# HAHHHD/mllp

Measured on AMD Instinct MI355X. Metric: LP instances/sec (fwd+bwd) on Netlib batch; achieved HBM GB/s on CSR SpMM, higher is better.
Workload: dtype f32; 1 GPU; netlib_full: BASELINE.json configs[2], 97 instances / 1,074,147 nnz per global batch, one block-diagonal batch per GPU, one Adam step per global batch: fwd + BCE + bwd + gradient all-reduce + Adam, fp32; global_batch=97, instances_rank0=97, nnz_rank0=1074147, hip_graph=False, parallelism=dp1

## Files before the change

mllp_amd/csrc/fused_kernels.hip:

```cpp
#include <algorithm>
#include <vector>

#include "device_utils.h"
#include "host_graph.h"
#include "internal.h"
#include "node_bodies.h"

namespace mllp {

typedef float f32x4m __attribute__((ext_vector_type(4)));

#ifdef MLLP_TIMING_BUILD
static int g_fused_abl = [] {
    const char* e = getenv("MLLP_FUSED_ABL");
    return e ? atoi(e) : 0;
}();
#define FUSED_ABL(bit) ((J.abl & (bit)) != 0)
__device__ unsigned long long g_fused_stamps[8192 * 8];
__device__ unsigned long long g_fused_stamps1[8192 * 8];
#define FUSED_STAMP(k)                                                                      \
    {                                                                                       \
        __builtin_amdgcn_sched_barrier(0);                                                  \
        const unsigned long long now_ = __builtin_amdgcn_s_memtime();                       \
        __builtin_amdgcn_sched_barrier(0);                                                  \
        stamp_sum[k] += now_ - stamp_last;                                                  \
        stamp_last = now_;                                                                  \
    }
#else
#define FUSED_ABL(bit) false
#define FUSED_STAMP(k)
#endif

constexpr int FT = 768;
constexpr int FW = FT / 64;
constexpr int RT = 1024;
constexpr int MAXJOBS = 2;

constexpr int NP = FUSED_NP;
static_assert(NP == FUSED_PARTS, "partition count");

struct PartTiers {
    int row0, n_block, n_wave, n_group, n_base;
};
struct ItemsDev {
    const int* __restrict__ sptr;
    const int2* __restrict__ sent;
    const float2* __restrict__ sax;
    int n_dst, nnz;
    const int* __restrict__ order;
    int nw, L;
    PartTiers part[NP];
};

static ItemsDev items_dev(const FusedOrient& o, int which) {
    const bool scalar = which == 1;
    ItemsDev d;
    d.order = which == 0 ? o.lst16 : which == 1 ? o.lst1 : o.lst16x2;
    d.nw = which == 0 ? o.nw16 : which == 1 ? o.nw1 : o.nw16x2;
    d.L = which == 0 ? o.L16 : which == 1 ? o.L1 : o.L16x2;
    d.sptr = o.sptr;
    d.sent = reinterpret_cast<const int2*>(o.sent);
    d.sax = reinterpret_cast<const float2*>(o.sax);
    d.n_dst = o.n_dst;
    d.nnz = o.nnz;
    for (int q = 0; q < NP; ++q) {
        const FusedTiersDev& t = scalar ? o.t1[q] : o.t16[q];
        d.part[q].row0 = o.row0[q];
        d.part[q].n_block = t.n_block; d.part[q].n_wave = t.n_wave; d.part[q].n_group = t.n_group; d.part[q].n_base = t.n_base;
    }
    return d;
}

constexpr int TS = 17;
constexpr int TILE = 16 * TS;
__device__ __forceinline__ void tile_put(float* tile, const float4& v, int lane) {
    float* d = tile + (lane >> 2) * TS + 4 * (lane & 3);
    d[0] = v.x; d[1] = v.y; d[2] = v.z; d[3] = v.w;
}
__device__ __forceinline__ float4 tile_get(const float* tile, int lane) {
    const float* d = tile + (lane >> 2) * TS + 4 * (lane & 3);
    return make_float4(d[0], d[1], d[2], d[3]);
}
__device__ __forceinline__ void tile_rows(const float* tile, int lane, float (&a)[4]) {
#pragma unroll
    for (int s = 0; s < 4; ++s) a[s] = tile[(lane & 15) * TS + 4 * s + (lane >> 4)];
}
__device__ __forceinline__ void tile_cols(const float* tile, int lane, float (&a)[4]) {
#pragma unroll
    for (int s = 0; s < 4; ++s) a[s] = tile[(4 * s + (lane >> 4)) * TS + (lane & 15)];
}
__device__ __forceinline__ void tile_put_result(float* tile, const f32x4m& d, int lane) {
#pragma unroll
    for (int j = 0; j < 4; ++j) tile[(4 * (lane >> 4) + j) * TS + (lane & 15)] = d[j];
}
struct MatB {
    float w[4];
};
__device__ __forceinline__ MatB matB(const float* __restrict__ W, int ld, int lane) {
    MatB b;
#pragma unroll
    for (int s = 0; s < 4; ++s) b.w[s] = W[(lane & 15) * ld + 4 * s + (lane >> 4)];
    return b;
}
__device__ __forceinline__ MatB matB_t(const float* __restrict__ W, int ld, int lane) {
    MatB b;
#pragma unroll
    for (int s = 0; s < 4; ++s) b.w[s] = W[(4 * s + (lane >> 4)) * ld + (lane & 15)];
    return b;
}
__device__ __forceinline__ void matB_store(float* lds, const MatB& b, int lane) {
    *reinterpret_cast<float4*>(lds + 4 * lane) = make_float4(b.w[0], b.w[1], b.w[2], b.w[3]);
}
__device__ __forceinline__ MatB matB_lds(const float* lds, int lane) {
    const float4 v = *reinterpret_cast<const float4*>(lds + 4 * lane);
    MatB b;
    b.w[0] = v.x; b.w[1] = v.y; b.w[2] = v.z; b.w[3] = v.w;
    return b;
}
__device__ __forceinline__ f32x4m mat_apply(const float (&a)[4], const MatB& b, f32x4m acc) {
#pragma unroll
    for (int s = 0; s < 4; ++s) acc = __builtin_amdgcn_mfma_f32_16x16x4f32(a[s], b.w[s], acc, 0, 0, 0);
    return acc;
}
__device__ __forceinline__ f32x4m splat4(float v) { return (f32x4m){v, v, v, v}; }
__device__ __forceinline__ float4 lds4(const float* p) { return *reinterpret_cast<const float4*>(p); }
__device__ __forceinline__ float4 f4zero() { return make_float4(0.f, 0.f, 0.f, 0.f); }
__device__ __forceinline__ float4 f4scale(const float4& a, float s) { return make_float4(a.x * s, a.y * s, a.z * s, a.w * s); }
__device__ __forceinline__ float4 f4add(const float4& a, const float4& b) { return make_float4(a.x + b.x, a.y + b.y, a.z + b.z, a.w + b.w); }
template <int J>
__device__ __forceinline__ int quad_bcast_i(int v) {
    return __builtin_amdgcn_mov_dpp(v, J * 0x55, 0xF, 0xF, true);
}
__device__ __forceinline__ float wave_sum(float v) {
    v = row16_sum(v);
    v += __shfl_xor(v, 16, 64);
    v += __shfl_xor(v, 32, 64);
    return v;
}


struct RowSlot {
    int row;
    int first;
    int stride;
    int end;
    int mode;
    bool writer;
};
struct SlotReq {
    int row, q, stride, mode;
    int sb, se;
    bool writer;
};
template <int G>
struct Geo {
    static constexpr int U = 64 / G;
    static constexpr int QG = 4;
    static constexpr int RG = U / QG;
};
template <int G>
__device__ __forceinline__ int wave_items(const PartTiers& s) {
    return s.n_wave + (s.n_group + Geo<G>::RG - 1) / Geo<G>::RG + (s.n_base + Geo<G>::U - 1) / Geo<G>::U;
}
template <int G>
__device__ __forceinline__ SlotReq item_request(const ItemsDev& S, const PartTiers& s, int item, int lane) {
    constexpr int U = Geo<G>::U, QG = Geo<G>::QG, RG = Geo<G>::RG;
    const int unit = lane / G;
    const int n_gitems = (s.n_group + RG - 1) / RG;
    SlotReq r;
    bool valid;
    if (item < s.n_wave) {
        r.row = s.row0 + s.n_block + item; r.q = unit; r.stride = U; r.mode = 2; valid = true; r.writer = unit == 0;
    } else if (item < s.n_wave + n_gitems) {
        const int rl = (item - s.n_wave) * RG + unit / QG;
        valid = rl < s.n_group;
        r.row = s.row0 + s.n_block + s.n_wave + rl; r.q = unit % QG; r.stride = QG; r.mode = 1; r.writer = valid && r.q == 0;
    } else {
        const int rl = (item - s.n_wave - n_gitems) * U + unit;
        valid = rl < s.n_base;
        r.row = s.row0 + s.n_block + s.n_wave + s.n_group + rl; r.q = 0; r.stride = 1; r.mode = 0; r.writer = valid;
    }
    const int rc = valid ? r.row : 0;
    r.sb = S.sptr[rc];
    r.se = S.sptr[rc + 1];
    if (!valid) r.row = -1;
    return r;
}
__device__ __forceinline__ SlotReq empty_request() {
    SlotReq r;
    r.row = -1; r.q = 0; r.stride = 1; r.mode = 0; r.sb = 0; r.se = 0; r.writer = false;
    return r;
}
__device__ __forceinline__ RowSlot slot_make(const SlotReq& q) {
    RowSlot r;
    r.row = q.row; r.first = q.sb + q.q; r.stride = q.stride; r.end = q.row >= 0 ? q.se : 0; r.mode = q.mode; r.writer = q.writer;
    asm volatile("" : "+v"(r.first), "+v"(r.end));
    return r;
}
template <int G>
__device__ __forceinline__ RowSlot item_slot(const ItemsDev& S, const PartTiers& s, int item, int lane) {
    return slot_make(item_request<G>(S, s, item, lane));
}
template <int G>
__device__ __forceinline__ RowSlot block_slot(const ItemsDev& s, int k, int tid) {
    RowSlot r;
    r.row = k;
    r.mode = 3;
    r.first = s.sptr[k] + tid / G;
    r.stride = FT / G;
    r.end = s.sptr[k + 1];
    r.writer = tid < G;
    return r;
}
__device__ __forceinline__ int slot_count(const RowSlot& r) {
    return r.first < r.end ? (r.end - r.first + r.stride - 1) / r.stride : 0;
}
__device__ __forceinline__ RowSlot empty_slot() {
    RowSlot r;
    r.row = -1; r.first = 0; r.stride = 1; r.end = 0; r.mode = 0; r.writer = false;
    return r;
}
struct WaveList {
    const int* p;
    int L, chunk;
};
__device__ __forceinline__ WaveList wave_list(const ItemsDev& S, int px, int gw) {
    WaveList w;
    w.L = gw < S.nw ? S.L : 0;
    w.p = S.order + ((size_t)px * S.nw + gw) * S.L;
    w.chunk = -1;
    return w;
}
__device__ __forceinline__ void wave_list_chunk(WaveList& w, int c0, int lane) {
    int v = c0 + lane < w.L ? w.p[c0 + lane] : -1;
    asm volatile("s_waitcnt vmcnt(0)" : "+v"(v));
    w.chunk = v;
}
__device__ __forceinline__ int wave_list_get(const WaveList& w, int k) {
    return k < 64 ? __builtin_amdgcn_readlane(w.chunk, __builtin_amdgcn_readfirstlane(k)) : -1;
}
template <int LPE>
__device__ __forceinline__ int2 first_entries(const ItemsDev& s, const RowSlot& r, int part) {
    const int k = LPE == 4 ? part : (part & 1);
    return k < slot_count(r) ? s.sent[r.first + k * r.stride] : make_int2(0, 0);
}
template <int LPE>
__device__ __forceinline__ int2 first_entries_any(const ItemsDev& s, const RowSlot& r, int part) {
    const int k = LPE == 4 ? part : (part & 1);
    return s.sent[max(min(r.first + k * r.stride, s.nnz - 1), 0)];
}
__device__ __forceinline__ float shared_sum4(float v, int mode) {
    return mode == 1 ? quads_sum<16>(v) : quads_sum<64>(v);
}
__device__ __forceinline__ float shared_max4(float v, int mode) {
    return mode == 1 ? quads_max<16>(v) : quads_max<64>(v);
}
__device__ __forceinline__ float shared_sum1(float v, int mode) { return mode == 1 ? quad_sum(v) : wave_sum(v); }
__device__ __forceinline__ float shared_max1(float v, int mode) { return mode == 1 ? quad_max(v) : group_max<64>(v); }

struct FwdJob16 {
    ItemsDev s;
    const float* __restrict__ x_src;
    const float* __restrict__ x_dst;
    const float* __restrict__ D;
    ConvParams p;
    float* __restrict__ h;
    float* __restrict__ Z;
    float* __restrict__ aux;
    int head;
    const float* __restrict__ fcw;
    const float* __restrict__ fcb;
    const float* __restrict__ inv_n;
    const float* __restrict__ labels;
    const int* __restrict__ perm;
    float inv_batch;
    float* __restrict__ logits;
    float* __restrict__ g_out;
    float* __restrict__ head_part;
#ifdef MLLP_TIMING_BUILD
    int abl;
#endif
};
struct FwdLaunch16 {
    FwdJob16 job[MAXJOBS];
    int n_jobs;
};
struct FwdW16 {
    float BPq[256], BWv[256], BWs[256];
    float pq0[16], Pt[16], bv[16], we[16], bs[16], fcw[16];
    float pt0, fcb;
};
struct SoftState {
    float4 Z;
    float m, L, u;
};

struct Gather4 {
    float4 x0, x1, x2, x3;
    float a0, a1, a2, a3;
};
__device__ __forceinline__ void gather4_issue(const ItemsDev& s, const float* __restrict__ X, const RowSlot& r, int n_mine,
                                              int k0, int part, int2& en, Gather4& g) {
    const int colm = en.x;
    const float am = __int_as_float(en.y);
    const int c0 = quad_bcast_i<0>(colm), c1 = quad_bcast_i<1>(colm), c2 = quad_bcast_i<2>(colm), c3 = quad_bcast_i<3>(colm);
    g.a0 = quad_bcast<0>(am); g.a1 = quad_bcast<1>(am); g.a2 = quad_bcast<2>(am); g.a3 = quad_bcast<3>(am);
    g.x0 = ld4(X + (size_t)c0 * 16 + 4 * part);
    g.x1 = ld4(X + (size_t)c1 * 16 + 4 * part);
    g.x2 = ld4(X + (size_t)c2 * 16 + 4 * part);
    g.x3 = ld4(X + (size_t)c3 * 16 + 4 * part);
    const int kn = k0 + 4 + part;
    en = kn < n_mine ? s.sent[r.first + kn * r.stride] : make_int2(0, 0);
}

__device__ __forceinline__ void fwd16_step(const Gather4& g, int k0, int n_mine, const float4& qp, float t, SoftState& st) {
    const bool ok0 = k0 < n_mine, ok1 = k0 + 1 < n_mine, ok2 = k0 + 2 < n_mine, ok3 = k0 + 3 < n_mine;
    const float d0 = ok0 ? fmaf(g.a0, t, quad_sum(dot4(qp, g.x0))) : NEG_BIG;
    const float d1 = ok1 ? fmaf(g.a1, t, quad_sum(dot4(qp, g.x1))) : NEG_BIG;
    const float d2 = ok2 ? fmaf(g.a2, t, quad_sum(dot4(qp, g.x2))) : NEG_BIG;
    const float d3 = ok3 ? fmaf(g.a3, t, quad_sum(dot4(qp, g.x3))) : NEG_BIG;
    const float mi = fmaxf(fmaxf(d0, d1), fmaxf(d2, d3));
    if (__any(mi > st.m)) {
        const float mn = fmaxf(st.m, mi);
        const float sc = exp_acc(st.m - mn);
        st.L *= sc; st.u *= sc;
        st.Z = f4scale(st.Z, sc);
        st.m = mn;
    }
    const float p0 = ok0 ? exp_acc(d0 - st.m) : 0.0f, p1 = ok1 ? exp_acc(d1 - st.m) : 0.0f;
    const float p2 = ok2 ? exp_acc(d2 - st.m) : 0.0f, p3 = ok3 ? exp_acc(d3 - st.m) : 0.0f;
    st.L += (p0 + p1) + (p2 + p3);
    st.u = fmaf(p0, g.a0, fmaf(p1, g.a1, fmaf(p2, g.a2, fmaf(p3, g.a3, st.u))));
    fma4(p0, g.x0, st.Z);
    fma4(p1, g.x1, st.Z);
    fma4(p2, g.x2, st.Z);
    fma4(p3, g.x3, st.Z);
}

__device__ __forceinline__ void soft_merge(SoftState& st, int mode) {
    const float M = shared_max4(st.m, mode);
    const float f = exp_acc(st.m - M);
    st.m = M;
    st.L = shared_sum4(st.L * f, mode);
    st.u = shared_sum4(st.u * f, mode);
    st.Z.x = shared_sum4(st.Z.x * f, mode);
    st.Z.y = shared_sum4(st.Z.y * f, mode);
    st.Z.z = shared_sum4(st.Z.z * f, mode);
    st.Z.w = shared_sum4(st.Z.w * f, mode);
}

struct HeadAcc {
    float4 w;
    float b, l;
};

struct FwdPending {
    float4 zn, hv, g, aux;
    float z;
    int row, lrow;
};
__device__ __forceinline__ void fwd16_flush(const FwdJob16& J, FwdPending& p, int part) {
    if (p.row >= 0 && !FUSED_ABL(2048)) {
        *reinterpret_cast<float4*>(J.Z + (size_t)p.row * 16 + 4 * part) = p.zn;
        if (part == 0) reinterpret_cast<float4*>(J.aux)[p.row] = p.aux;
        if (J.head != 2) *reinterpret_cast<float4*>(J.h + (size_t)p.row * 16 + 4 * part) = p.hv;
        if (J.head && part == 0) J.logits[p.lrow] = p.z;
        if (J.head == 2) *reinterpret_cast<float4*>(J.g_out + (size_t)p.row * 16 + 4 * part) = p.g;
    }
    p.row = -1;
}

struct FwdNext {
    RowSlot r;
    float4 xd;
    int2 en;
    int lrow;
    SlotReq q;
};
__device__ __forceinline__ void fwd16_row(const FwdJob16& J, const FwdW16& W, const PartTiers& P, const RowSlot& r,
                                          const float4& xd, int2& en, int lrow, const SlotReq& q1, int it2, FwdNext& nx,
                                          FwdPending& pend, int part, int lane, float* merge_lds, float* tiles, HeadAcc& ha
#ifdef MLLP_TIMING_BUILD
                                          , unsigned long long (&stamp_sum)[8], unsigned long long& stamp_last
#endif
) {
    FUSED_STAMP(0)
    const int n_mine = FUSED_ABL(256) ? 0 : slot_count(r);
    Gather4 gt;
    gather4_issue(J.s, J.x_src, r, n_mine, 0, part, en, gt);
    nx.r = slot_make(q1);
    nx.xd = ld4(J.x_dst + (size_t)max(nx.r.row, 0) * 16 + 4 * part);
    nx.en = first_entries_any<4>(J.s, nx.r, part);
    nx.lrow = J.perm[max(nx.r.row, 0)];
    nx.q = item_request<4>(J.s, P, max(it2, 0), lane);
    float4 qp;
    float t;
    {
        float ax_[4];
        tile_put(tiles, xd, lane);
        tile_rows(tiles, lane, ax_);
        if (!FUSED_ABL(1024))
        tile_put_result(tiles + TILE, mat_apply(ax_, matB_lds(W.BPq, lane), splat4(W.pq0[lane & 15])), lane);
        qp = tile_get(tiles + TILE, lane);
        t = quad_sum(dot4(lds4(W.Pt + 4 * part), xd)) + W.pt0;
    }
    FUSED_STAMP(1)
    SoftState st;
    st.Z = f4zero(); st.m = NEG_BIG; st.L = 0.0f; st.u = 0.0f;
    for (int k0 = 0;;) {
        fwd16_step(gt, k0, n_mine, qp, t, st);
        k0 += 4;
        if (!__any(k0 < n_mine)) break;
        gather4_issue(J.s, J.x_src, r, n_mine, k0, part, en, gt);
    }
    FUSED_STAMP(2)
    asm volatile("" : "+v"(nx.xd.x), "+v"(nx.xd.y), "+v"(nx.xd.z), "+v"(nx.xd.w), "+v"(nx.en.x), "+v"(nx.en.y),
                      "+v"(nx.lrow), "+v"(nx.q.sb), "+v"(nx.q.se));
    fwd16_flush(J, pend, part);
    const int lrow_cur = lrow;
    FUSED_STAMP(3)

    if (r.mode >= 1) soft_merge(st, r.mode);
    if (r.mode == 3) {
        const int wave = threadIdx.x >> 6;
        if (lane < 4) {
            float* slot = merge_lds + wave * 20;
            if (part == 0) *reinterpret_cast<float4*>(slot) = make_float4(st.m, st.L, st.u, 0.0f);
            *reinterpret_cast<float4*>(slot + 4 + 4 * part) = st.Z;
        }
        __syncthreads();
        float M = NEG_BIG;
        for (int w = 0; w < FW; ++w) M = fmaxf(M, merge_lds[w * 20]);
        float L = 0.0f, u = 0.0f;
        float4 Z = f4zero();
        for (int w = 0; w < FW; ++w) {
            const float4 hd = lds4(merge_lds + w * 20);
            const float f = exp_acc(hd.x - M);
            L = fmaf(f, hd.y, L);
            u = fmaf(f, hd.z, u);
            fma4(f, lds4(merge_lds + w * 20 + 4 + 4 * part), Z);
        }
        st.m = M; st.L = L; st.u = u; st.Z = Z;
        __syncthreads();
    }
    const bool writer = r.writer;
    const float rinv = 1.0f / (st.L + 1e-16f);
    const float S = st.L * rinv, un = st.u * rinv;
    const float4 zn = f4scale(st.Z, rinv);
    float4 o;
    {
        float ax_[4], az_[4];
        tile_rows(tiles, lane, ax_);
        tile_put(tiles + TILE, zn, lane);
        tile_rows(tiles + TILE, lane, az_);
        if (!FUSED_ABL(512))
        tile_put_result(tiles + 2 * TILE,
                        mat_apply(ax_, matB_lds(W.BWs, lane), mat_apply(az_, matB_lds(W.BWv, lane), splat4(0.0f))), lane);
        o = tile_get(tiles + 2 * TILE, lane);
    }
    o = f4add(o, lds4(W.bs + 4 * part));
    fma4(S, lds4(W.bv + 4 * part), o);
    fma4(un, lds4(W.we + 4 * part), o);
    const float4 hv = make_float4(fmaxf(o.x, 0.0f), fmaxf(o.y, 0.0f), fmaxf(o.z, 0.0f), fmaxf(o.w, 0.0f));
    FUSED_STAMP(4)
    pend.row = writer ? r.row : -1;
    pend.zn = zn; pend.hv = hv; pend.lrow = lrow_cur;
    pend.aux = make_float4(un, st.L > 0.0f ? st.m : 0.0f, rinv, S);
    pend.z = 0.0f; pend.g = f4zero();
    if (J.head) {
        const float4 fw = lds4(W.fcw + 4 * part);
        const float z = quad_sum(dot4(hv, fw)) + W.fcb;
        pend.z = z;
        if (J.head == 2 && writer) {
            const float y = J.labels[r.row];
            const float wn = J.inv_n[r.row] * J.inv_batch;
            const float e = expf(-fabsf(z));
            const float sig = z >= 0.0f ? 1.0f / (1.0f + e) : e / (1.0f + e);
            const float dz = wn * (sig - y);
            pend.g = make_float4(hv.x > 0.0f ? dz * fw.x : 0.0f, hv.y > 0.0f ? dz * fw.y : 0.0f,
                                 hv.z > 0.0f ? dz * fw.z : 0.0f, hv.w > 0.0f ? dz * fw.w : 0.0f);
            fma4(dz, hv, ha.w);
            if (part == 0) {
                ha.b += dz;
                ha.l += wn * (fmaxf(z, 0.0f) - z * y + log1pf(e));
            }
        }
    }
    FUSED_STAMP(5)
}

template <int NW>
__device__ __forceinline__ void head_partials_store(HeadAcc& ha, float* head_lds, float* head_part, int tid) {
    const int lane = tid & 63, wave = tid >> 6;
    ha.w.x = quads_sum<64>(ha.w.x); ha.w.y = quads_sum<64>(ha.w.y);
    ha.w.z = quads_sum<64>(ha.w.z); ha.w.w = quads_sum<64>(ha.w.w);
    ha.b = wave_sum(ha.b);
    ha.l = wave_sum(ha.l);
    if (lane < 4) {
        float* d = head_lds + wave * 18 + 4 * lane;
        d[0] = ha.w.x; d[1] = ha.w.y; d[2] = ha.w.z; d[3] = ha.w.w;
    }
    if (lane == 0) { head_lds[wave * 18 + 16] = ha.b; head_lds[wave * 18 + 17] = ha.l; }
    __syncthreads();
    if (tid < 18) {
        float v = 0.0f;
        for (int w = 0; w < NW; ++w) v += head_lds[w * 18 + tid];
        head_part[(size_t)blockIdx.x * 18 + tid] = v;
    }
}

__global__ __launch_bounds__(FT) void fused_fwd16_kernel(FwdLaunch16 A) {
    __shared__ FwdW16 Ws_[MAXJOBS];
    __shared__ float merge_lds[FW * 20];
    __shared__ float head_lds[FW * 18];
    __shared__ float tiles_[FW * 3 * TILE];
    const int tid = threadIdx.x, lane = tid & 63, wave = tid >> 6, part = lane & 3;
    for (int j = 0; j < A.n_jobs; ++j) {
        const FwdJob16& J = A.job[j];
        FwdW16& W = Ws_[j];
        if (wave == 0) matB_store(W.BPq, matB(J.D + OFF_PQ, 16, lane), lane);
        if (wave == 1) matB_store(W.BWv, matB(J.p.Wv, 16, lane), lane);
        if (wave == 2) matB_store(W.BWs, matB(J.p.Ws, 16, lane), lane);
        if (tid < 16) {
            W.pq0[tid] = J.D[OFF_PQ0 + tid];
            W.Pt[tid] = J.D[OFF_PT + tid];
            W.bv[tid] = J.p.bv[tid];
            W.we[tid] = J.p.we[tid];
            W.bs[tid] = J.p.bs[tid];
            W.fcw[tid] = J.head ? J.fcw[tid] : 0.0f;
        }
        if (tid == 0) {
            W.pt0 = J.D[OFF_PT0];
            W.fcb = J.head ? J.fcb[0] : 0.0f;
        }
    }
    __syncthreads();
    float* tiles = tiles_ + wave * 3 * TILE;
    HeadAcc ha;
    ha.w = f4zero(); ha.b = 0.0f; ha.l = 0.0f;
#ifdef MLLP_TIMING_BUILD
    unsigned long long stamp_sum[8] = {0, 0, 0, 0, 0, 0, 0, 0};
    unsigned long long stamp_last = __builtin_amdgcn_s_memtime();
    const unsigned long long stamp_begin = stamp_last;
#define STAMP_ARGS , stamp_sum, stamp_last
#else
#define STAMP_ARGS
#endif
    const int px = blockIdx.x % NP, bi = blockIdx.x / NP, gp = gridDim.x / NP;
    const int gw = bi * FW + wave;
    float* head_part = nullptr;
    for (int j = 0; j < A.n_jobs; ++j) {
        const FwdJob16& J = A.job[j];
        const PartTiers P = J.s.part[px];
        if (J.head == 2) head_part = J.head_part;
        const RowSlot none = empty_slot();
        FwdPending pend;
        pend.row = -1;
        for (int k = bi; k < P.n_block; k += gp) {
            const RowSlot r = block_slot<4>(J.s, P.row0 + k, tid);
            const float4 xd = ld4(J.x_dst + (size_t)r.row * 16 + 4 * part);
            int2 en = first_entries<4>(J.s, r, part);
            const int lrow = J.head ? J.perm[r.row] : 0;
            FwdNext nx;
            fwd16_row(J, Ws_[j], P, r, xd, en, lrow, empty_request(), -1, nx, pend, part, lane, merge_lds, tiles, ha STAMP_ARGS);
        }
        WaveList wl = wave_list(J.s, px, gw);
        for (int c0 = 0; c0 < wl.L; c0 += 64) {
            wave_list_chunk(wl, c0, lane);
            int it = wave_list_get(wl, 0), it1 = wave_list_get(wl, 1);
            RowSlot r = it >= 0 ? item_slot<4>(J.s, P, it, lane) : none;
            float4 xd = r.row >= 0 ? ld4(J.x_dst + (size_t)r.row * 16 + 4 * part) : f4zero();
            int2 en = first_entries<4>(J.s, r, part);
            int lrow = (J.head && r.row >= 0) ? J.perm[r.row] : 0;
            SlotReq q1 = item_request<4>(J.s, P, max(it1, 0), lane);
            if (it1 < 0) q1.row = -1;
            asm volatile("" : "+v"(xd.x), "+v"(xd.y), "+v"(xd.z), "+v"(xd.w), "+v"(en.x), "+v"(en.y), "+v"(lrow),
                              "+v"(q1.sb), "+v"(q1.se));
            for (int k = 0; it >= 0; ++k) {
                const int it2 = wave_list_get(wl, k + 2);
                FwdNext nx;
                fwd16_row(J, Ws_[j], P, r, xd, en, lrow, q1, it2, nx, pend, part, lane, merge_lds, tiles, ha STAMP_ARGS);
#ifdef MLLP_TIMING_BUILD
                stamp_sum[7] += 1;
#endif
                r = nx.r; xd = nx.xd; en = nx.en; lrow = nx.lrow; q1 = nx.q;
                it = it1; it1 = it2;
            }
        }
        fwd16_flush(J, pend, part);
    }
#ifdef MLLP_TIMING_BUILD
    if (lane == 0 && A.job[0].abl >= 0) {
        stamp_sum[6] = __builtin_amdgcn_s_memtime() - stamp_begin;
        unsigned long long* d = g_fused_stamps + (size_t)(blockIdx.x * FW + wave) * 8;
        for (int k = 0; k < 8; ++k) d[k] = stamp_sum[k];
    }
#endif
    if (head_part) head_partials_store<FW>(ha, head_lds, head_part, tid);
}

struct FwdJob1 {
    ItemsDev s;
    const float* __restrict__ x_dst;
    const float* __restrict__ D;
    ConvParams p;
    float* __restrict__ h;
    float* __restrict__ Z;
    float* __restrict__ aux;
};
struct FwdLaunch1 {
    FwdJob1 job[MAXJOBS];
    int n_jobs;
};
struct alignas(16) FwdW1 {
    float wv[16], ws[16], bv[16], we[16], bs[16];
    float pq, pq0, pt, pt0;
};
struct Soft1 {
    float m, L, u, Z;
};

struct Ent8 {
    float2 e0, e1, e2, e3, e4, e5, e6, e7;
};
__device__ __forceinline__ void ent8_load(const ItemsDev& s, const RowSlot& r, int k0, Ent8& E) {
    const int last = max(s.nnz - 1, 0), d = r.stride, b = r.first + k0 * d;
    E.e0 = s.sax[min(b, last)];         E.e1 = s.sax[min(b + d, last)];
    E.e2 = s.sax[min(b + 2 * d, last)]; E.e3 = s.sax[min(b + 3 * d, last)];
    E.e4 = s.sax[min(b + 4 * d, last)]; E.e5 = s.sax[min(b + 5 * d, last)];
    E.e6 = s.sax[min(b + 6 * d, last)]; E.e7 = s.sax[min(b + 7 * d, last)];
}

__device__ __forceinline__ void fwd1_step4(const float2& e0, const float2& e1, const float2& e2, const float2& e3, int k0,
                                           int n_mine, float qp, float t, Soft1& st) {
    const bool ok0 = k0 < n_mine, ok1 = k0 + 1 < n_mine, ok2 = k0 + 2 < n_mine, ok3 = k0 + 3 < n_mine;
    const float d0 = ok0 ? fmaf(qp, e0.y, e0.x * t) : NEG_BIG, d1 = ok1 ? fmaf(qp, e1.y, e1.x * t) : NEG_BIG;
    const float d2 = ok2 ? fmaf(qp, e2.y, e2.x * t) : NEG_BIG, d3 = ok3 ? fmaf(qp, e3.y, e3.x * t) : NEG_BIG;
    const float mi = fmaxf(fmaxf(d0, d1), fmaxf(d2, d3));
    if (__any(mi > st.m)) {
        const float mn = fmaxf(st.m, mi);
        const float sc = exp_acc(st.m - mn);
        st.L *= sc; st.u *= sc; st.Z *= sc;
        st.m = mn;
    }
    const float p0 = ok0 ? exp_acc(d0 - st.m) : 0.0f, p1 = ok1 ? exp_acc(d1 - st.m) : 0.0f;
    const float p2 = ok2 ? exp_acc(d2 - st.m) : 0.0f, p3 = ok3 ? exp_acc(d3 - st.m) : 0.0f;
    st.L += (p0 + p1) + (p2 + p3);
    st.u = fmaf(p0, e0.x, fmaf(p1, e1.x, fmaf(p2, e2.x, fmaf(p3, e3.x, st.u))));
    st.Z = fmaf(p0, e0.y, fmaf(p1, e1.y, fmaf(p2, e2.y, fmaf(p3, e3.y, st.Z))));
}
__device__ __forceinline__ void fwd1_edges(const ItemsDev& s, const RowSlot& r, float qp, float t, Soft1& st, Ent8& E) {
    const int n_mine = slot_count(r);
    for (int k0 = 0; __any(k0 < n_mine); k0 += 8) {
        Ent8 N;
        const bool more = __any(k0 + 8 < n_mine);
        if (more) ent8_load(s, r, k0 + 8, N);
        fwd1_step4(E.e0, E.e1, E.e2, E.e3, k0, n_mine, qp, t, st);
        if (__any(k0 + 4 < n_mine)) fwd1_step4(E.e4, E.e5, E.e6, E.e7, k0 + 4, n_mine, qp, t, st);
        if (more) E = N;
    }
}

__device__ __forceinline__ void fwd1_row(const FwdJob1& J, const FwdW1& W, const RowSlot& r, int lane, float* merge_lds) {
    Ent8 E;
    ent8_load(J.s, r, 0, E);
    const float x = J.x_dst[max(r.row, 0)];
    const float qp = fmaf(W.pq, x, W.pq0), t = fmaf(W.pt, x, W.pt0);
    Soft1 st;
    st.m = NEG_BIG; st.L = 0.0f; st.u = 0.0f; st.Z = 0.0f;
    fwd1_edges(J.s, r, qp, t, st, E);
    if (r.mode >= 1) {
        const float M = shared_max1(st.m, r.mode);
        const float f = exp_acc(st.m - M);
        st.m = M;
        st.L = shared_sum1(st.L * f, r.mode);
        st.u = shared_sum1(st.u * f, r.mode);
        st.Z = shared_sum1(st.Z * f, r.mode);
    }
    if (r.mode == 3) {
        const int wave = threadIdx.x >> 6;
        if (lane == 0) *reinterpret_cast<float4*>(merge_lds + wave * 4) = make_float4(st.m, st.L, st.u, st.Z);
        __syncthreads();
        float M = NEG_BIG;
        for (int w = 0; w < FW; ++w) M = fmaxf(M, merge_lds[w * 4]);
        float L = 0.0f, u = 0.0f, Z = 0.0f;
        for (int w = 0; w < FW; ++w) {
            const float4 hd = lds4(merge_lds + w * 4);
            const float f = exp_acc(hd.x - M);
            L = fmaf(f, hd.y, L);
            u = fmaf(f, hd.z, u);
            Z = fmaf(f, hd.w, Z);
        }
        st.m = M; st.L = L; st.u = u; st.Z = Z;
        __syncthreads();
    }
    const float rinv = 1.0f / (st.L + 1e-16f);
    const float S = st.L * rinv, un = st.u * rinv, zn = st.Z * rinv;
    if (r.mode == 0) {
        const int base_row = __builtin_amdgcn_readfirstlane(r.row);
        const int n_valid = __popcll(__ballot(r.row >= 0));
#pragma unroll
        for (int q = 0; q < 4; ++q) {
            const int idx = lane + 64 * q, row_l = idx >> 2, ch = (idx & 3) * 4;
            const float Sr = __shfl(S, row_l, 64), ur = __shfl(un, row_l, 64), zr = __shfl(zn, row_l, 64), xr = __shfl(x, row_l, 64);
            float4 v = lds4(W.bs + ch);
            fma4(Sr, lds4(W.bv + ch), v);
            fma4(ur, lds4(W.we + ch), v);
            fma4(zr, lds4(W.wv + ch), v);
            fma4(xr, lds4(W.ws + ch), v);
            if (row_l < n_valid)
                *reinterpret_cast<float4*>(J.h + (size_t)(base_row + row_l) * 16 + ch) =
                    make_float4(fmaxf(v.x, 0.0f), fmaxf(v.y, 0.0f), fmaxf(v.z, 0.0f), fmaxf(v.w, 0.0f));
        }
        if (r.writer) {
            J.Z[r.row] = zn;
            reinterpret_cast<float4*>(J.aux)[r.row] = make_float4(un, st.L > 0.0f ? st.m : 0.0f, rinv, S);
        }
        return;
    }
    if (!r.writer) return;
    float o[16];
#pragma unroll
    for (int c = 0; c < 16; ++c) {
        float v = W.bs[c];
        v = fmaf(S, W.bv[c], v);
        v = fmaf(un, W.we[c], v);
        v = fmaf(W.wv[c], zn, v);
        v = fmaf(W.ws[c], x, v);
        o[c] = fmaxf(v, 0.0f);
    }
    float4* hd = reinterpret_cast<float4*>(J.h + (size_t)r.row * 16);
    hd[0] = make_float4(o[0], o[1], o[2], o[3]);
    hd[1] = make_float4(o[4], o[5], o[6], o[7]);
    hd[2] = make_float4(o[8], o[9], o[10], o[11]);
    hd[3] = make_float4(o[12], o[13], o[14], o[15]);
    J.Z[r.row] = zn;
    reinterpret_cast<float4*>(J.aux)[r.row] = make_float4(un, st.L > 0.0f ? st.m : 0.0f, rinv, S);
}

__global__ __launch_bounds__(FT) void fused_fwd1_kernel(FwdLaunch1 A) {
    __shared__ FwdW1 Ws_[MAXJOBS];
    __shared__ float merge_lds[FW * 4];
    const int tid = threadIdx.x, lane = tid & 63, wave = tid >> 6;
    for (int j = 0; j < A.n_jobs; ++j) {
        const FwdJob1& J = A.job[j];
        FwdW1& W = Ws_[j];
        if (tid < 16) {
            W.wv[tid] = J.p.Wv[tid]; W.ws[tid] = J.p.Ws[tid];
            W.bv[tid] = J.p.bv[tid]; W.we[tid] = J.p.we[tid]; W.bs[tid] = J.p.bs[tid];
        }
        if (tid == 0) {
            W.pq = J.D[OFF_PQ]; W.pq0 = J.D[OFF_PQ0]; W.pt = J.D[OFF_PT]; W.pt0 = J.D[OFF_PT0];
        }
    }
    __syncthreads();
    const int px = blockIdx.x % NP, bi = blockIdx.x / NP, gp = gridDim.x / NP;
    const int gw = bi * FW + wave;
    for (int j = 0; j < A.n_jobs; ++j) {
        const FwdJob1& J = A.job[j];
        const PartTiers P = J.s.part[px];
        for (int k = bi; k < P.n_block; k += gp)
            fwd1_row(J, Ws_[j], block_slot<1>(J.s, P.row0 + k, tid), lane, merge_lds);
        WaveList wl = wave_list(J.s, px, gw);
        for (int c0 = 0; c0 < wl.L; c0 += 64) {
            wave_list_chunk(wl, c0, lane);
            int it = wave_list_get(wl, 0);
            SlotReq q = item_request<1>(J.s, P, max(it, 0), lane);
            for (int k = 0; it >= 0; ++k) {
                const int itn = wave_list_get(wl, k + 1);
                const RowSlot r = slot_make(q);
                q = item_request<1>(J.s, P, max(itn, 0), lane);
                fwd1_row(J, Ws_[j], r, lane, merge_lds);
                it = itn;
            }
        }
    }
}

struct BwdJob16 {
    ItemsDev s;
    const float* __restrict__ x_src;
    const float* __restrict__ x_dst;
    const float* __restrict__ D;
    ConvParams p;
    const float* __restrict__ h;
    const float* __restrict__ dh_a;
    const float* __restrict__ dh_b;
    const float* __restrict__ Z;
    const float* __restrict__ aux;
    float* __restrict__ rec;
    float* __restrict__ dx_dst;
    int mask_dx;
    float* __restrict__ stats;
#ifdef MLLP_TIMING_BUILD
    int abl;
#endif
};
struct BwdLaunch16 {
    BwdJob16 job[MAXJOBS];
    int n_jobs;
};
struct BwdW16 {
    float BWvT[256], BPq[256], BWsT[256], BPqT[256];
    float pq0[16], Pt[16], Pb[16], bv[16], we[16];
    float pt0;
};
struct BwdState {
    float4 dq;
    float ds, dt;
};

__device__ __forceinline__ void bwd16_step(const Gather4& g, int k0, int n_mine, const float4& qp, const float4& gv, float t,
                                           float m, float rinv, float ge, float cc, BwdState& st) {
#define MLLP_BWD_SLOT(K, A_, X_)                                                           \
    {                                                                                      \
        const float l_ = fmaf(A_, t, quad_sum(dot4(qp, X_)));                              \
        const float al_ = (k0 + K < n_mine) ? exp_acc(l_ - m) * rinv : 0.0f;               \
        const float dl_ = al_ * (quad_sum(dot4(gv, X_)) + fmaf(A_, ge, cc));               \
        st.ds += dl_;                                                                      \
        st.dt = fmaf(dl_, A_, st.dt);                                                      \
        fma4(dl_, X_, st.dq);                                                              \
    }
    MLLP_BWD_SLOT(0, g.a0, g.x0)
    MLLP_BWD_SLOT(1, g.a1, g.x1)
    MLLP_BWD_SLOT(2, g.a2, g.x2)
    MLLP_BWD_SLOT(3, g.a3, g.x3)
#undef MLLP_BWD_SLOT
}

struct BwdRow {
    float4 ga, gb, h, x, Z, ax;
};
__device__ __forceinline__ void bwd16_fetch(const BwdJob16& J, const RowSlot& r, int part, BwdRow& d) {
    const bool have = r.row >= 0;
    const size_t ro = have ? (size_t)r.row * 16 + 4 * part : 0;
    const float4 z4 = f4zero();
    d.ga = have ? ld4(J.dh_a + ro) : z4;
    d.gb = (J.dh_b && have) ? ld4(J.dh_b + ro) : z4;
    d.h = (J.h && have) ? ld4(J.h + ro) : make_float4(1.0f, 1.0f, 1.0f, 1.0f);
    d.x = have ? ld4(J.x_dst + ro) : z4;
    d.Z = have ? ld4(J.Z + ro) : z4;
    d.ax = have ? reinterpret_cast<const float4*>(J.aux)[r.row] : z4;
}

constexpr int TB_G = 0, TB_X = 1, TB_Z = 2, TB_DQ = 3, TB_SC = 4, TB_E = 5, TB_N = 6;

__device__ __forceinline__ void bwd16_row(const BwdJob16& J, const BwdW16& W, const PartTiers& P, const RowSlot& r,
                                          BwdRow& rd, int2& en, int itn, RowSlot& rn, int part,
                                          int lane, float* merge_lds, float* tiles, f32x4m (&acc)[STAT_TILES]) {
    const bool have = r.row >= 0;
    const bool writer = r.writer;
    const int n_mine = FUSED_ABL(1) ? 0 : slot_count(r);
    Gather4 gt;
    gather4_issue(J.s, J.x_src, r, n_mine, 0, part, en, gt);
    SlotReq qn = item_request<4>(J.s, P, max(itn, 0), lane);
    if (itn < 0) qn.row = -1;
    const int xpos = (rd.x.x > 0.0f ? 1 : 0) | (rd.x.y > 0.0f ? 2 : 0) | (rd.x.z > 0.0f ? 4 : 0) | (rd.x.w > 0.0f ? 8 : 0);
    float4 qp, gv;
    float t, m, rinv, ge, cc;
    {
        float4 g = f4add(rd.ga, rd.gb);
        g = make_float4(rd.h.x > 0.0f ? g.x : 0.0f, rd.h.y > 0.0f ? g.y : 0.0f, rd.h.z > 0.0f ? g.z : 0.0f, rd.h.w > 0.0f ? g.w : 0.0f);
        const float4 xd = rd.x, Zn = rd.Z, ax = rd.ax;
        float ag_[4], ax_[4];
        tile_put(tiles + TB_G * TILE, g, lane);
        tile_put(tiles + TB_X * TILE, xd, lane);
        tile_put(tiles + TB_Z * TILE, Zn, lane);
        tile_put(tiles + TB_E * TILE, (have && part == 0) ? make_float4(1.0f, ax.w, ax.x, 0.0f) : f4zero(), lane);
        tile_rows(tiles + TB_G * TILE, lane, ag_);
        tile_rows(tiles + TB_X * TILE, lane, ax_);
        if (!FUSED_ABL(16)) {
            tile_put_result(tiles + TB_DQ * TILE, mat_apply(ag_, matB_lds(W.BWvT, lane), splat4(0.0f)), lane);
            tile_put_result(tiles + TB_SC * TILE, mat_apply(ax_, matB_lds(W.BPq, lane), splat4(W.pq0[lane & 15])), lane);
        }
        gv = tile_get(tiles + TB_DQ * TILE, lane);
        qp = tile_get(tiles + TB_SC * TILE, lane);
        t = quad_sum(dot4(lds4(W.Pt + 4 * part), xd)) + W.pt0;
        ge = quad_sum(dot4(g, lds4(W.we + 4 * part)));
        const float gb = quad_sum(dot4(g, lds4(W.bv + 4 * part)));
        const float Dn = quad_sum(dot4(gv, Zn)) + gb * ax.w + ge * ax.x;
        cc = gb - Dn;
        m = ax.y; rinv = ax.z;
    }
    BwdState st;
    st.dq = f4zero(); st.ds = 0.0f; st.dt = 0.0f;
    for (int k0 = 0;;) {
        bwd16_step(gt, k0, n_mine, qp, gv, t, m, rinv, ge, cc, st);
        k0 += 4;
        if (!__any(k0 < n_mine)) break;
        gather4_issue(J.s, J.x_src, r, n_mine, k0, part, en, gt);
    }
    if (writer && J.rec && !FUSED_ABL(8)) {
        float* rr = J.rec + (size_t)r.row * REC_W;
        *reinterpret_cast<float4*>(rr + 4 * part) = qp;
        *reinterpret_cast<float4*>(rr + 16 + 4 * part) = gv;
        if (part == 0) *reinterpret_cast<float4*>(rr + 32) = make_float4(t, m, rinv, ge);
        if (part == 1) *reinterpret_cast<float4*>(rr + 36) = make_float4(cc, 0.0f, 0.0f, 0.0f);
    }
    rn = slot_make(qn);
    bwd16_fetch(J, rn, part, rd);
    en = first_entries<4>(J.s, rn, part);
    if (r.mode >= 1) {
        st.ds = shared_sum4(st.ds, r.mode);
        st.dt = shared_sum4(st.dt, r.mode);
        st.dq.x = shared_sum4(st.dq.x, r.mode); st.dq.y = shared_sum4(st.dq.y, r.mode);
        st.dq.z = shared_sum4(st.dq.z, r.mode); st.dq.w = shared_sum4(st.dq.w, r.mode);
    }
    if (r.mode == 3) {
        const int wave = threadIdx.x >> 6;
        if (lane < 4) {
            float* slot = merge_lds + wave * 20;
            if (part == 0) *reinterpret_cast<float4*>(slot) = make_float4(st.ds, st.dt, 0.0f, 0.0f);
            *reinterpret_cast<float4*>(slot + 4 + 4 * part) = st.dq;
        }
        __syncthreads();
        float ds = 0.0f, dt = 0.0f;
        float4 dq = f4zero();
        for (int w = 0; w < FW; ++w) {
            ds += merge_lds[w * 20];
            dt += merge_lds[w * 20 + 1];
            dq = f4add(dq, lds4(merge_lds + w * 20 + 4 + 4 * part));
        }
        st.ds = ds; st.dt = dt; st.dq = dq;
        __syncthreads();
        if (threadIdx.x >= 64) return;
    }
    tile_put(tiles + TB_DQ * TILE, st.dq, lane);
    if (J.dx_dst && !FUSED_ABL(4)) {
        float ag_[4], adq_[4];
        tile_rows(tiles + TB_G * TILE, lane, ag_);
        tile_rows(tiles + TB_DQ * TILE, lane, adq_);
        tile_put_result(tiles + TB_SC * TILE,
                        mat_apply(adq_, matB_lds(W.BPqT, lane), mat_apply(ag_, matB_lds(W.BWsT, lane), splat4(0.0f))), lane);
        float4 v = tile_get(tiles + TB_SC * TILE, lane);
        fma4(st.ds, lds4(W.Pb + 4 * part), v);
        fma4(st.dt, lds4(W.Pt + 4 * part), v);
        if (J.mask_dx) {
            if (!(xpos & 1)) v.x = 0.0f;
            if (!(xpos & 2)) v.y = 0.0f;
            if (!(xpos & 4)) v.z = 0.0f;
            if (!(xpos & 8)) v.w = 0.0f;
        }
        if (writer) *reinterpret_cast<float4*>(J.dx_dst + (size_t)r.row * 16 + 4 * part) = v;
    }
    if (FUSED_ABL(2)) return;
    if (r.mode >= 1 && !writer) {
        const float4 z4 = f4zero();
        tile_put(tiles + TB_G * TILE, z4, lane);
        tile_put(tiles + TB_X * TILE, z4, lane);
        tile_put(tiles + TB_Z * TILE, z4, lane);
        tile_put(tiles + TB_E * TILE, z4, lane);
        tile_put(tiles + TB_DQ * TILE, z4, lane);
    }
    tile_put(tiles + TB_SC * TILE, (writer && part == 0) ? make_float4(st.ds, st.dt, 0.0f, 0.0f) : f4zero(), lane);
    float cg[4], cdq[4], csc[4], cx[4], cz[4], ce[4];
    if (FUSED_ABL(64)) {
        for (int s = 0; s < 4; ++s) { cg[s] = cdq[s] = csc[s] = cx[s] = cz[s] = ce[s] = (float)lane; }
    } else {
    tile_cols(tiles + TB_G * TILE, lane, cg);
    tile_cols(tiles + TB_DQ * TILE, lane, cdq);
    tile_cols(tiles + TB_SC * TILE, lane, csc);
    tile_cols(tiles + TB_X * TILE, lane, cx);
    tile_cols(tiles + TB_Z * TILE, lane, cz);
    tile_cols(tiles + TB_E * TILE, lane, ce);
    }
    if (FUSED_ABL(32)) {
        asm volatile("" :: "v"(cg[0]), "v"(cdq[1]), "v"(csc[2]), "v"(cx[3]), "v"(cz[0]), "v"(ce[1]));
        return;
    }
#pragma unroll
    for (int s = 0; s < 4; ++s) {
        acc[0] = __builtin_amdgcn_mfma_f32_16x16x4f32(cg[s], cx[s], acc[0], 0, 0, 0);
        acc[1] = __builtin_amdgcn_mfma_f32_16x16x4f32(cg[s], cz[s], acc[1], 0, 0, 0);
        acc[2] = __builtin_amdgcn_mfma_f32_16x16x4f32(cg[s], ce[s], acc[2], 0, 0, 0);
        acc[3] = __builtin_amdgcn_mfma_f32_16x16x4f32(cdq[s], cx[s], acc[3], 0, 0, 0);
        acc[4] = __builtin_amdgcn_mfma_f32_16x16x4f32(cdq[s], ce[s], acc[4], 0, 0, 0);
        acc[5] = __builtin_amdgcn_mfma_f32_16x16x4f32(csc[s], cx[s], acc[5], 0, 0, 0);
        acc[6] = __builtin_amdgcn_mfma_f32_16x16x4f32(csc[s], ce[s], acc[6], 0, 0, 0);
    }
}

__global__ __launch_bounds__(FT) void fused_bwd16_kernel(BwdLaunch16 A) {
    __shared__ BwdW16 Ws_[MAXJOBS];
    __shared__ float merge_lds[FW * 20];
    __shared__ float tiles_[FW * TB_N * TILE];
    const int tid = threadIdx.x, lane = tid & 63, wave = tid >> 6, part = lane & 3;
    for (int j = 0; j < A.n_jobs; ++j) {
        const BwdJob16& J = A.job[j];
        BwdW16& W = Ws_[j];
        if (wave == 0) matB_store(W.BWvT, matB_t(J.p.Wv, 16, lane), lane);
        if (wave == 1) matB_store(W.BPq, matB(J.D + OFF_PQ, 16, lane), lane);
        if (wave == 2) matB_store(W.BWsT, matB_t(J.p.Ws, 16, lane), lane);
        if (wave == 3) matB_store(W.BPqT, matB_t(J.D + OFF_PQ, 16, lane), lane);
        if (tid < 16) {
            W.pq0[tid] = J.D[OFF_PQ0 + tid];
            W.Pt[tid] = J.D[OFF_PT + tid];
            W.Pb[tid] = J.D[OFF_PB + tid];
            W.bv[tid] = J.p.bv[tid];
            W.we[tid] = J.p.we[tid];
        }
        if (tid == 0) W.pt0 = J.D[OFF_PT0];
    }
    __syncthreads();
    float* tiles = tiles_ + wave * TB_N * TILE;
    const int px = blockIdx.x % NP, bi = blockIdx.x / NP, gp = gridDim.x / NP;
    const int gw = bi * FW + wave;
    for (int j = 0; j < A.n_jobs; ++j) {
        const BwdJob16& J = A.job[j];
        const PartTiers P = J.s.part[px];
        f32x4m acc[STAT_TILES];
#pragma unroll
        for (int i = 0; i < STAT_TILES; ++i) acc[i] = splat4(0.0f);
        const RowSlot none = empty_slot();
        for (int k = bi; k < P.n_block; k += gp) {
            const RowSlot r = block_slot<4>(J.s, P.row0 + k, tid);
            BwdRow rd;
            bwd16_fetch(J, r, part, rd);
            int2 en = first_entries<4>(J.s, r, part);
            RowSlot rn;
            bwd16_row(J, Ws_[j], P, r, rd, en, -1, rn, part, lane, merge_lds, tiles, acc);
        }
        WaveList wl = wave_list(J.s, px, gw);
        for (int c0 = 0; c0 < wl.L; c0 += 64) {
            wave_list_chunk(wl, c0, lane);
            int it = wave_list_get(wl, 0);
            RowSlot r = it >= 0 ? item_slot<4>(J.s, P, it, lane) : none;
            BwdRow rd;
            bwd16_fetch(J, r, part, rd);
            int2 en = first_entries<4>(J.s, r, part);
            for (int k = 0; it >= 0; ++k) {
                const int itn = wave_list_get(wl, k + 1);
                RowSlot rn;
                bwd16_row(J, Ws_[j], P, r, rd, en, itn, rn, part, lane, merge_lds, tiles, acc);
                r = rn;
                it = itn;
            }
        }
        __syncthreads();
        float* red = tiles_;
#pragma unroll
        for (int i = 0; i < STAT_TILES; ++i) {
#pragma unroll
            for (int q = 0; q < 4; ++q) red[wave * 256 + ((lane >> 4) * 4 + q) * 16 + (lane & 15)] = acc[i][q];
            __syncthreads();
            if (tid < 256) {
                float v = 0.0f;
                for (int w = 0; w < FW; ++w) v += red[w * 256 + tid];
                J.stats[(size_t)blockIdx.x * STAT_FLOATS + i * 256 + tid] = v;
            }
            __syncthreads();
        }
    }
}

struct SrcJob16 {
    ItemsDev s;
    const float* __restrict__ x;
    const float* __restrict__ rec;
    float* __restrict__ dx;
    const float* __restrict__ addp;
    float addw;
    int mask;
};
struct SrcLaunch16 {
    SrcJob16 job[MAXJOBS];
    int n_jobs;
};

__device__ __forceinline__ void src16_row(const SrcJob16& J, const RowSlot& r, float4& xj_io, int2& en, const SlotReq& qn,
                                          RowSlot& rn, int part, int lane, float* merge_lds) {
    const int n_mine = slot_count(r);
    const float4 xj = xj_io;
    const float4 addv = ld4(J.addp + (size_t)max(r.row, 0) * 16 + 4 * part);
    float4 acc = f4zero();
    for (int k0 = 0; __any(k0 < n_mine); k0 += 2) {
        const int colm = en.x;
        const float am = __int_as_float(en.y);
        const int c0 = quad_bcast_i<0>(colm), c1 = quad_bcast_i<1>(colm);
        const float a0 = quad_bcast<0>(am), a1 = quad_bcast<1>(am);
        const bool ok0 = k0 < n_mine, ok1 = k0 + 1 < n_mine;
        const float* rr0 = J.rec + (size_t)c0 * REC_W;
        const float* rr1 = J.rec + (size_t)c1 * REC_W;
        const float4 q0 = ld4(rr0 + 4 * part), g0 = ld4(rr0 + 16 + 4 * part), s0 = ld4(rr0 + 32);
        const float cc0 = rr0[36];
        const float4 q1 = ld4(rr1 + 4 * part), g1 = ld4(rr1 + 16 + 4 * part), s1 = ld4(rr1 + 32);
        const float cc1 = rr1[36];
        const int kn = k0 + 2 + (part & 1);
        en = kn < n_mine ? J.s.sent[r.first + kn * r.stride] : make_int2(0, 0);
        {
            const float l = fmaf(a0, s0.x, quad_sum(dot4(q0, xj)));
            const float al = ok0 ? exp_acc(l - s0.y) * s0.z : 0.0f;
            const float dl = al * (quad_sum(dot4(g0, xj)) + fmaf(a0, s0.w, cc0));
            fma4(al, g0, acc);
            fma4(dl, q0, acc);
        }
        {
            const float l = fmaf(a1, s1.x, quad_sum(dot4(q1, xj)));
            const float al = ok1 ? exp_acc(l - s1.y) * s1.z : 0.0f;
            const float dl = al * (quad_sum(dot4(g1, xj)) + fmaf(a1, s1.w, cc1));
            fma4(al, g1, acc);
            fma4(dl, q1, acc);
        }
    }
    rn = slot_make(qn);
    xj_io = rn.row >= 0 ? ld4(J.x + (size_t)rn.row * 16 + 4 * part) : f4zero();
    en = first_entries<2>(J.s, rn, part);
    if (r.mode >= 1) {
        acc.x = shared_sum4(acc.x, r.mode); acc.y = shared_sum4(acc.y, r.mode);
        acc.z = shared_sum4(acc.z, r.mode); acc.w = shared_sum4(acc.w, r.mode);
    }
    if (r.mode == 3) {
        const int wave = threadIdx.x >> 6;
        if (lane < 4) *reinterpret_cast<float4*>(merge_lds + wave * 20 + 4 * part) = acc;
        __syncthreads();
        float4 v = f4zero();
        for (int w = 0; w < FW; ++w) v = f4add(v, lds4(merge_lds + w * 20 + 4 * part));
        acc = v;
        __syncthreads();
    }
    fma4(J.addw, addv, acc);
    if (J.mask) {
        if (!(xj.x > 0.0f)) acc.x = 0.0f;
        if (!(xj.y > 0.0f)) acc.y = 0.0f;
        if (!(xj.z > 0.0f)) acc.z = 0.0f;
        if (!(xj.w > 0.0f)) acc.w = 0.0f;
    }
    if (r.writer) *reinterpret_cast<float4*>(J.dx + (size_t)r.row * 16 + 4 * part) = acc;
}

__global__ __launch_bounds__(FT) void fused_src16_kernel(SrcLaunch16 A) {
    __shared__ float merge_lds[FW * 20];
    const int tid = threadIdx.x, lane = tid & 63, wave = tid >> 6, part = lane & 3;
    const int px = blockIdx.x % NP, bi = blockIdx.x / NP, gp = gridDim.x / NP;
    const int gw = bi * FW + wave;
    for (int j = 0; j < A.n_jobs; ++j) {
        const SrcJob16& J = A.job[j];
        const PartTiers P = J.s.part[px];
        const RowSlot none = empty_slot();
        for (int k = bi; k < P.n_block; k += gp) {
            const RowSlot r = block_slot<4>(J.s, P.row0 + k, tid);
            float4 xj = ld4(J.x + (size_t)r.row * 16 + 4 * part);
            int2 en = first_entries<2>(J.s, r, part);
            RowSlot rn;
            src16_row(J, r, xj, en, empty_request(), rn, part, lane, merge_lds);
        }
        WaveList wl = wave_list(J.s, px, gw);
        for (int c0 = 0; c0 < wl.L; c0 += 64) {
            wave_list_chunk(wl, c0, lane);
            int it = wave_list_get(wl, 0);
            RowSlot r = it >= 0 ? item_slot<4>(J.s, P, it, lane) : none;
            float4 xj = r.row >= 0 ? ld4(J.x + (size_t)r.row * 16 + 4 * part) : f4zero();
            int2 en = first_entries<2>(J.s, r, part);
            for (int k = 0; it >= 0; ++k) {
                const int itn = wave_list_get(wl, k + 1);
                const SlotReq qn = itn >= 0 ? item_request<4>(J.s, P, itn, lane) : empty_request();
                RowSlot rn;
                src16_row(J, r, xj, en, qn, rn, part, lane, merge_lds);
                r = rn;
                it = itn;
            }
        }
    }
}

struct BwdJob1 {
    ItemsDev s;
    const float* __restrict__ x_dst;
    const float* __restrict__ D;
    ConvParams p;
    const float* __restrict__ g;
    const float* __restrict__ Z;
    const float* __restrict__ aux;
    float* __restrict__ stats;
};
struct BwdLaunch1 {
    BwdJob1 job[MAXJOBS];
    int n_jobs;
};
struct alignas(16) BwdW1 {
    float wv[16], bv[16], we[16];
    float pq, pq0, pt, pt0;
};
constexpr int G1S = 17, R1S = 9;
constexpr int TILE1 = 64 * G1S + 64 * R1S;

__device__ __forceinline__ void bwd1_row(const BwdJob1& J, const BwdW1& W, const RowSlot& r, int lane, float* merge_lds,
                                         float* tiles, f32x4m& accT, float (&accS)[6]
#ifdef MLLP_TIMING_BUILD
                                         , unsigned long long (&stamp_sum)[8], unsigned long long& stamp_last
#endif
) {
    FUSED_STAMP(0)
    const bool writer = r.writer;
    Ent8 E;
    ent8_load(J.s, r, 0, E);
    const int rowc = max(r.row, 0);
    float gv = 0.0f, ge = 0.0f, gb = 0.0f;
    if (r.mode == 0) {
        const int base_row = __builtin_amdgcn_readfirstlane(r.row);
        const int n_valid = __popcll(__ballot(r.row >= 0));
        float* gt = tiles;
        float* rt = tiles + 64 * G1S;
#pragma unroll
        for (int q = 0; q < 4; ++q) {
            const int idx = lane + 64 * q, row_l = idx >> 2, ch = (idx & 3) * 4;
            const size_t ro = (size_t)min(base_row + row_l, J.s.n_dst - 1) * 16 + ch;
            const float4 a = ld4(J.g + ro);
            const bool on = row_l < n_valid;
            const float4 g = make_float4(on ? a.x : 0.0f, on ? a.y : 0.0f, on ? a.z : 0.0f, on ? a.w : 0.0f);
            const float pv = quad_sum(dot4(g, lds4(W.wv + ch))), pe = quad_sum(dot4(g, lds4(W.we + ch)));
            const float pb = quad_sum(dot4(g, lds4(W.bv + ch)));
            float* d = gt + row_l * G1S + ch;
            d[0] = g.x; d[1] = g.y; d[2] = g.z; d[3] = g.w;
            if ((lane & 3) == 0) { rt[row_l * R1S + 5] = pv; rt[row_l * R1S + 6] = pe; rt[row_l * R1S + 7] = pb; }
        }
        gv = rt[lane * R1S + 5]; ge = rt[lane * R1S + 6]; gb = rt[lane * R1S + 7];
    } else {
        const float4* pa = reinterpret_cast<const float4*>(J.g + (size_t)rowc * 16);
        float* gt = tiles + lane * G1S;
#pragma unroll
        for (int q = 0; q < 4; ++q) {
            const float4 a = pa[q];
            const float g0 = a.x, g1 = a.y, g2 = a.z, g3 = a.w;
            gv = fmaf(g0, W.wv[4 * q], fmaf(g1, W.wv[4 * q + 1], fmaf(g2, W.wv[4 * q + 2], fmaf(g3, W.wv[4 * q + 3], gv))));
            ge = fmaf(g0, W.we[4 * q], fmaf(g1, W.we[4 * q + 1], fmaf(g2, W.we[4 * q + 2], fmaf(g3, W.we[4 * q + 3], ge))));
            gb = fmaf(g0, W.bv[4 * q], fmaf(g1, W.bv[4 * q + 1], fmaf(g2, W.bv[4 * q + 2], fmaf(g3, W.bv[4 * q + 3], gb))));
            gt[4 * q] = writer ? g0 : 0.0f;
            gt[4 * q + 1] = writer ? g1 : 0.0f;
            gt[4 * q + 2] = writer ? g2 : 0.0f;
            gt[4 * q + 3] = writer ? g3 : 0.0f;
        }
    }
    const float x = J.x_dst[rowc];
    const float Zn = J.Z[rowc];
    const float4 ax = reinterpret_cast<const float4*>(J.aux)[rowc];
    {
        float* rt = tiles + 64 * G1S + lane * R1S;
        rt[0] = writer ? x : 0.0f;
        rt[1] = writer ? Zn : 0.0f;
        rt[2] = writer ? 1.0f : 0.0f;
        rt[3] = writer ? ax.w : 0.0f;
        rt[4] = writer ? ax.x : 0.0f;
    }
    const float Dn = gv * Zn + gb * ax.w + ge * ax.x;
    const float cc = gb - Dn;
    const float qp = fmaf(W.pq, x, W.pq0), t = fmaf(W.pt, x, W.pt0);
    float ds = 0.0f, dt = 0.0f, dq = 0.0f;
    const int n_mine = slot_count(r);
    FUSED_STAMP(1)
    for (int k0 = 0; __any(k0 < n_mine); k0 += 8) {
        Ent8 N;
        const bool more = __any(k0 + 8 < n_mine);
        if (more) ent8_load(J.s, r, k0 + 8, N);
#define MLLP_BWD1_SLOT(K, E_)                                                              \
    {                                                                                      \
        const float l_ = fmaf(qp, E_.y, E_.x * t);                                         \
        const float al_ = (K) < n_mine ? exp_acc(l_ - ax.y) * ax.z : 0.0f;                 \
        const float dl_ = al_ * fmaf(gv, E_.y, fmaf(E_.x, ge, cc));                        \
        ds += dl_;                                                                         \
        dt = fmaf(dl_, E_.x, dt);                                                          \
        dq = fmaf(dl_, E_.y, dq);                                                          \
    }
        MLLP_BWD1_SLOT(k0, E.e0)
        MLLP_BWD1_SLOT(k0 + 1, E.e1)
        MLLP_BWD1_SLOT(k0 + 2, E.e2)
        MLLP_BWD1_SLOT(k0 + 3, E.e3)
        if (__any(k0 + 4 < n_mine)) {
            MLLP_BWD1_SLOT(k0 + 4, E.e4)
            MLLP_BWD1_SLOT(k0 + 5, E.e5)
            MLLP_BWD1_SLOT(k0 + 6, E.e6)
            MLLP_BWD1_SLOT(k0 + 7, E.e7)
        }
#undef MLLP_BWD1_SLOT
        if (more) E = N;
    }
    FUSED_STAMP(2)
    if (r.mode >= 1) {
        ds = shared_sum1(ds, r.mode); dt = shared_sum1(dt, r.mode); dq = shared_sum1(dq, r.mode);
    }
    if (r.mode == 3) {
        const int wave = threadIdx.x >> 6;
        if (lane == 0) *reinterpret_cast<float4*>(merge_lds + wave * 4) = make_float4(ds, dt, dq, 0.0f);
        __syncthreads();
        float a = 0.0f, b = 0.0f, c = 0.0f;
        for (int w = 0; w < FW; ++w) {
            const float4 v = lds4(merge_lds + w * 4);
            a += v.x; b += v.y; c += v.z;
        }
        ds = a; dt = b; dq = c;
        __syncthreads();
        if (threadIdx.x >= 64) return;
    }
    if (writer) {
        accS[0] = fmaf(dq, x, accS[0]);
        accS[1] += dq;
        accS[2] = fmaf(ds, x, accS[2]);
        accS[3] = fmaf(dt, x, accS[3]);
        accS[4] += ds;
        accS[5] += dt;
    }
    FUSED_STAMP(3)
    const float* gt = tiles;
    const float* rt = tiles + 64 * G1S;
    const int kq = lane >> 4, rr = lane & 15;
#pragma unroll
    for (int s = 0; s < 16; ++s) {
        const float a = gt[(4 * s + kq) * G1S + rr];
        const float b = rr < 5 ? rt[(4 * s + kq) * R1S + rr] : 0.0f;
        accT = __builtin_amdgcn_mfma_f32_16x16x4f32(a, b, accT, 0, 0, 0);
    }
    FUSED_STAMP(4)
}

__global__ __launch_bounds__(FT) void fused_bwd1_kernel(BwdLaunch1 A) {
    __shared__ BwdW1 Ws_[MAXJOBS];
    __shared__ float merge_lds[FW * 4];
    __shared__ float tiles_[FW * TILE1];
    const int tid = threadIdx.x, lane = tid & 63, wave = tid >> 6;
    for (int j = 0; j < A.n_jobs; ++j) {
        const BwdJob1& J = A.job[j];
        BwdW1& W = Ws_[j];
        if (tid < 16) { W.wv[tid] = J.p.Wv[tid]; W.bv[tid] = J.p.bv[tid]; W.we[tid] = J.p.we[tid]; }
        if (tid == 0) { W.pq = J.D[OFF_PQ]; W.pq0 = J.D[OFF_PQ0]; W.pt = J.D[OFF_PT]; W.pt0 = J.D[OFF_PT0]; }
    }
    __syncthreads();
    float* tiles = tiles_ + wave * TILE1;
    const int px = blockIdx.x % NP, bi = blockIdx.x / NP, gp = gridDim.x / NP;
    const int gw = bi * FW + wave;
#ifdef MLLP_TIMING_BUILD
    unsigned long long stamp_sum[8] = {0, 0, 0, 0, 0, 0, 0, 0};
    unsigned long long stamp_last = __builtin_amdgcn_s_memtime();
    const unsigned long long stamp_begin = stamp_last;
#define STAMP_ARGS1 , stamp_sum, stamp_last
#else
#define STAMP_ARGS1
#endif
    for (int j = 0; j < A.n_jobs; ++j) {
        const BwdJob1& J = A.job[j];
        const PartTiers P = J.s.part[px];
        f32x4m accT = splat4(0.0f);
        float accS[6] = {0.0f, 0.0f, 0.0f, 0.0f, 0.0f, 0.0f};
        for (int k = bi; k < P.n_block; k += gp)
            bwd1_row(J, Ws_[j], block_slot<1>(J.s, P.row0 + k, tid), lane, merge_lds, tiles, accT, accS STAMP_ARGS1);
        WaveList wl = wave_list(J.s, px, gw);
        for (int c0 = 0; c0 < wl.L; c0 += 64) {
            wave_list_chunk(wl, c0, lane);
            int it = wave_list_get(wl, 0);
            SlotReq q = item_request<1>(J.s, P, max(it, 0), lane);
            for (int k = 0; it >= 0; ++k) {
                const int itn = wave_list_get(wl, k + 1);
                const RowSlot r = slot_make(q);
                q = item_request<1>(J.s, P, max(itn, 0), lane);
                bwd1_row(J, Ws_[j], r, lane, merge_lds, tiles, accT, accS STAMP_ARGS1);
#ifdef MLLP_TIMING_BUILD
                stamp_sum[7] += 1;
#endif
                it = itn;
            }
        }
        __syncthreads();
        float* red = tiles_;
#pragma unroll
        for (int q = 0; q < 4; ++q) red[wave * 262 + ((lane >> 4) * 4 + q) * 16 + (lane & 15)] = accT[q];
#pragma unroll
        for (int i = 0; i < 6; ++i) {
            const float v = wave_sum(accS[i]);
            if (lane == 0) red[wave * 262 + 256 + i] = v;
        }
        __syncthreads();
        float* dst = J.stats + (size_t)blockIdx.x * STAT_FLOATS;
        for (int i = tid; i < STAT_FLOATS; i += FT) dst[i] = 0.0f;
        __syncthreads();
        if (tid < 262) {
            float v = 0.0f;
            for (int w = 0; w < FW; ++w) v += red[w * 262 + tid];
            const int o = tid >> 4, n = tid & 15;
            if (tid >= 256) {
                const int i = tid - 256;
                const int slot = i == 0 ? 768 : i == 1 ? 1024 : i == 2 ? 1280 : i == 3 ? 1280 + 16 : i == 4 ? 1536 : 1536 + 16;
                dst[slot] = v;
            } else if (n == 0) dst[o * 16] = v;
            else if (n == 1) dst[256 + o * 16] = v;
            else if (n < 5) dst[512 + o * 16 + (n - 2)] = v;
        }
        __syncthreads();
#ifdef MLLP_TIMING_BUILD
        stamp_last = __builtin_amdgcn_s_memtime();
#endif
    }
#ifdef MLLP_TIMING_BUILD
    if (lane == 0) {
        stamp_sum[6] = __builtin_amdgcn_s_memtime() - stamp_begin;
        unsigned long long* d = g_fused_stamps1 + (size_t)(blockIdx.x * FW + wave) * 8;
        for (int k = 0; k < 8; ++k) d[k] = stamp_sum[k];
    }
#endif
#undef STAMP_ARGS1
}

__global__ __launch_bounds__(RT) void fused_head_bwd_kernel(int n, const float* __restrict__ h3, const float* __restrict__ fcw,
                                                            const float* __restrict__ dlogits, const int* __restrict__ perm,
                                                            float* __restrict__ dh3, float* __restrict__ head_part) {
    __shared__ float head_lds[(RT / 64) * 18];
    const int tid = threadIdx.x, lane = tid & 63, part = lane & 3;
    HeadAcc ha;
    ha.w = f4zero(); ha.b = 0.0f; ha.l = 0.0f;
    const float4 fw = ld4(fcw + 4 * part);
    for (int row = blockIdx.x * (RT / 4) + (tid >> 2); row < n; row += gridDim.x * (RT / 4)) {
        const float dz = dlogits[perm[row]];
        const float4 hv = ld4(h3 + (size_t)row * 16 + 4 * part);
        *reinterpret_cast<float4*>(dh3 + (size_t)row * 16 + 4 * part) = f4scale(fw, dz);
        fma4(dz, hv, ha.w);
        if (part == 0) ha.b += dz;
    }
    head_partials_store<RT / 64>(ha, head_lds, head_part, tid);
}

struct ReduceArgs {
    const float* stats[MODEL_CONVS];
    float* out[MODEL_CONVS];
    int nblk;
    const float* head_part;
    float* head_out;
    float* loss_out;
};

__device__ __forceinline__ void fused_reduce_body(const ReduceArgs& A, int n_conv) {
    __shared__ float sh[32][32];
    const int tid = threadIdx.x;
    if ((int)blockIdx.x == n_conv * STAT_TILES) {
        if (!A.head_part) return;
        const int col = tid & 31, slice = tid >> 5;
        float v = 0.0f;
        if (col < 18)
            for (int b = slice; b < A.nblk; b += 32) v += A.head_part[(size_t)b * 18 + col];
        sh[slice][col] = v;
        __syncthreads();
        if (tid < 18) {
            float t = 0.0f;
            for (int q = 0; q < 32; ++q) t += sh[q][tid];
            if (tid < 17) A.head_out[tid] = t;
            else if (A.loss_out) A.loss_out[0] = t;
        }
        return;
    }
    float* sh4 = &sh[0][0];
    const int col = tid & 255, slice = tid >> 8;
    const int c = blockIdx.x / STAT_TILES, tile = blockIdx.x % STAT_TILES;
    const float* src = A.stats[c] + tile * 256 + col;
    float v = 0.0f;
    int b = slice;
    for (; b + 124 < A.nblk; b += 128) {
        float t[32];
#pragma unroll
        for (int q = 0; q < 32; ++q) t[q] = src[(size_t)(b + 4 * q) * STAT_FLOATS];
#pragma unroll
        for (int q = 0; q < 32; ++q) v += t[q];
    }
    for (; b + 28 < A.nblk; b += 32) {
        float t[8];
#pragma unroll
        for (int q = 0; q < 8; ++q) t[q] = src[(size_t)(b + 4 * q) * STAT_FLOATS];
#pragma unroll
        for (int q = 0; q < 8; ++q) v += t[q];
    }
    for (; b < A.nblk; b += 4) v += src[(size_t)b * STAT_FLOATS];
    sh4[slice * 256 + col] = v;
    __syncthreads();
    if (tid < 256) A.out[c][tile * 256 + tid] = (sh4[tid] + sh4[256 + tid]) + (sh4[512 + tid] + sh4[768 + tid]);
}
__global__ __launch_bounds__(RT) void fused_reduce_kernel(ReduceArgs A, int n_conv) { fused_reduce_body(A, n_conv); }

struct TailArgs {
    ReduceArgs R;
    ConvParams p[MODEL_CONVS];
    int cin[MODEL_CONVS];
    float* grads[MODEL_CONVS];
    float* zero;
    int n_zero;
    float* params; const float* grads_all; float* m; float* v; float* state;
    float eps;
    int n_params;
    float* D[MODEL_CONVS];
    unsigned long long* sync;
    unsigned* err;
};
__device__ __forceinline__ bool tail_barrier(unsigned long long* cnt, unsigned long long target, unsigned* err_host) {
    __shared__ int ok_s;
    unsigned long long* err_dev = cnt + 2;
    __syncthreads();
    if (threadIdx.x == 0) {
        __threadfence();
        __hip_atomic_fetch_add(cnt, 1ull, __ATOMIC_RELEASE, __HIP_MEMORY_SCOPE_AGENT);
        int spins = 0;
        while (__hip_atomic_load(cnt, __ATOMIC_ACQUIRE, __HIP_MEMORY_SCOPE_AGENT) < target && ++spins < (1 << 22))
            __builtin_amdgcn_s_sleep(8);
        if (spins >= (1 << 22)) {
            __hip_atomic_store(err_dev, 1ull, __ATOMIC_RELAXED, __HIP_MEMORY_SCOPE_AGENT);
            __hip_atomic_store(err_host, 1u, __ATOMIC_RELAXED, __HIP_MEMORY_SCOPE_SYSTEM);
        }
        __threadfence();
        ok_s = __hip_atomic_load(err_dev, __ATOMIC_RELAXED, __HIP_MEMORY_SCOPE_AGENT) == 0ull;
    }
    __syncthreads();
    return ok_s != 0;
}
__global__ __launch_bounds__(RT) void fused_tail_kernel(TailArgs A, int n_conv) {
    const unsigned long long G = gridDim.x, epoch = A.sync[1];
    const int b = blockIdx.x;
    const float step = A.state[0] + 1.0f, lr = A.state[1], b1 = A.state[2], b2 = A.state[3];
    fused_reduce_body(A.R, n_conv);
    if (!tail_barrier(A.sync, (epoch + 1) * G, A.err)) return;
    if (b < n_conv) {
        finalize_conv_body(A.cin[b], A.p[b], A.R.out[b], 1, A.grads[b]);
        __syncthreads();
        const int off = (int)(A.grads[b] - A.grads_all), n = 4 * FEAT * A.cin[b] + 5 * FEAT;
        adam_slice(A.params + off, A.grads_all + off, A.m + off, A.v + off, step, lr, b1, b2, A.eps, 1.0f, n);
        __syncthreads();
        if (threadIdx.x < BLOCK) param_prep_body(A.p[b], A.cin[b], A.D[b]);
    } else if (b == n_conv) {
        for (int k = threadIdx.x; k < A.n_zero; k += RT) A.zero[k] = 0.0f;
        const int off = (int)(A.R.head_out - A.grads_all);
        adam_slice(A.params + off, A.grads_all + off, A.m + off, A.v + off, step, lr, b1, b2, A.eps, 1.0f, A.n_params - off);
        if (threadIdx.x == 0) {
            A.state[0] = step;
            A.sync[1] = epoch + 1;
        }
    }
}

__global__ __launch_bounds__(256) void fused_fill_kernel(int n_dst, const int* __restrict__ perm, const int* __restrict__ ptr,
                                                         const int* __restrict__ idx, const float* __restrict__ val,
                                                         const int* __restrict__ inv_src, const int* __restrict__ sptr,
                                                         int2* __restrict__ sent) {
    const int k = blockIdx.x * 4 + (threadIdx.x >> 6), lane = threadIdx.x & 63;
    if (k >= n_dst) return;
    const int r = perm[k], beg = ptr[r], deg = ptr[r + 1] - beg, o = sptr[k];
    for (int e = lane; e < deg; e += 64) sent[o + e] = make_int2(inv_src[idx[beg + e]], __float_as_int(val[beg + e]));
}
__global__ void fused_permute_kernel(int n, const int* __restrict__ perm, const float* __restrict__ src, float* __restrict__ dst) {
    for (int i = blockIdx.x * blockDim.x + threadIdx.x; i < n; i += gridDim.x * blockDim.x) dst[i] = src[perm[i]];
}
__global__ void fused_pregather_kernel(int64_t nnz, const int2* __restrict__ sent, const float* __restrict__ xs,
                                       float2* __restrict__ sax) {
    for (int64_t e = blockIdx.x * (int64_t)blockDim.x + threadIdx.x; e < nnz; e += (int64_t)gridDim.x * blockDim.x) {
        const int2 v = sent[e];
        sax[e] = make_float2(__int_as_float(v.y), xs[v.x]);
    }
}

#ifdef MLLP_TIMING_BUILD
extern "C" int mllp_timing_read_stamps(unsigned long long* host, int n) {
    return hipMemcpyFromSymbol(host, HIP_SYMBOL(g_fused_stamps), (size_t)n * sizeof(unsigned long long)) == hipSuccess ? 0 : -1;
}
extern "C" int mllp_timing_read_stamps1(unsigned long long* host, int n) {
    return hipMemcpyFromSymbol(host, HIP_SYMBOL(g_fused_stamps1), (size_t)n * sizeof(unsigned long long)) == hipSuccess ? 0 : -1;
}
#endif

static int check_launch(const char* what) {
    hipError_t e = hipGetLastError();
    return e == hipSuccess ? MLLP_OK : hip_fail(e, what);
}

template <class T>
static int dev_alloc(mllp_graph* g, size_t count, T** out, const T* host = nullptr) {
    void* p = nullptr;
    MLLP_HIP_TRY(hipMalloc(&p, std::max<size_t>(count, 1) * sizeof(T)));
    g->allocs.push_back(p);
    if (host && count) MLLP_HIP_TRY(hipMemcpy(p, host, count * sizeof(T), hipMemcpyHostToDevice));
    *out = static_cast<T*>(p);
    return MLLP_OK;
}

static void set_tiers(FusedTiersDev& d, const FusedTiers& t) {
    d.n_block = t.n_block; d.n_wave = t.n_wave; d.n_group = t.n_group; d.n_base = t.n_base;
}

int fused_refill_values(mllp_graph* g, hipStream_t s) {
    int rc;
    if (g->M > 0) {
        hipLaunchKernelGGL(fused_fill_kernel, dim3((unsigned)((g->M + 3) / 4)), dim3(256), 0, s, (int)g->M, g->perm_c, g->A.ptr,
                           g->A.idx, g->A.val, g->inv_v, g->FA.sptr, reinterpret_cast<int2*>(g->FA.sent));
        if ((rc = check_launch("fused_fill A"))) return rc;
    }
    if (g->N > 0) {
        hipLaunchKernelGGL(fused_fill_kernel, dim3((unsigned)((g->N + 3) / 4)), dim3(256), 0, s, (int)g->N, g->perm_v, g->At.ptr,
                           g->At.idx, g->At.val, g->inv_c, g->FAt.sptr, reinterpret_cast<int2*>(g->FAt.sent));
        if ((rc = check_launch("fused_fill At"))) return rc;
    }
    return MLLP_OK;
}

int fused_graph_build(mllp_graph* g, const int* h_csr_ptr, const int* h_csc_ptr) {
    if (g->fused_built) return MLLP_OK;
    if ((int64_t)g->h_csr_ptr.size() != g->M + 1 && !h_csr_ptr) return fail(MLLP_EINVAL, "fused path: no host row pointers");
    HostFusedOrient hc, hv;
    {
#ifdef MLLP_SCALAR_PARTITION
        const std::vector<int> part = host_partition_instances(host_instance_cost(h_csr_ptr, g->h_inst_ptr_m),
                                                               host_instance_cost(h_csc_ptr, g->h_inst_ptr_n), FUSED_PARTS);
#else
        const std::vector<int> part = host_partition_instances_v(host_instance_loads(h_csr_ptr, g->h_inst_ptr_m),
                                                                 host_instance_loads(h_csc_ptr, g->h_inst_ptr_n), FUSED_PARTS);
#endif
        host_build_fused_orient(h_csr_ptr, (int)g->M, g->h_inst_ptr_m, part, &hc);
        host_build_fused_orient(h_csc_ptr, (int)g->N, g->h_inst_ptr_n, part, &hv);
    }
    int rc;
    if ((rc = dev_alloc(g, (size_t)g->M, &g->perm_c, hc.perm.data()))) return rc;
    if ((rc = dev_alloc(g, (size_t)g->N, &g->perm_v, hv.perm.data()))) return rc;
    if ((rc = dev_alloc(g, (size_t)g->M, &g->inv_c, hc.inv.data()))) return rc;
    if ((rc = dev_alloc(g, (size_t)g->N, &g->inv_v, hv.inv.data()))) return rc;
    FusedOrient& A = g->FA;
    FusedOrient& At = g->FAt;
    A.n_dst = (int)g->M; A.n_src = (int)g->N; A.nnz = (int)g->nnz;
    At.n_dst = (int)g->N; At.n_src = (int)g->M; At.nnz = (int)g->nnz;
    for (int q = 0; q < NP; ++q) {
        set_tiers(A.t16[q], hc.t16[q]); set_tiers(A.t1[q], hc.t1[q]);
        set_tiers(At.t16[q], hv.t16[q]); set_tiers(At.t1[q], hv.t1[q]);
    }
    for (int q = 0; q <= NP; ++q) { A.row0[q] = hc.row0[q]; At.row0[q] = hv.row0[q]; }
    {
        const int gp = fused_grid(g) / NP;
        const HostFusedOrient* ho[2] = {&hc, &hv};
        FusedOrient* dv[2] = {&A, &At};
        for (int k = 0; k < 2; ++k) {
            HostWaveLists l16, l16x2, l1;
            host_build_wave_lists(*ho[k], false, gp * FW, FW, 4, &l16);
            host_build_wave_lists(*ho[k], false, 2 * gp * FW, FW, 2, &l16x2);
            host_build_wave_lists(*ho[k], true, gp * FW, FW, 8, &l1);
            FusedOrient& d = *dv[k];
            d.L16 = l16.L; d.nw16 = l16.waves_per_part;
            d.L16x2 = l16x2.L; d.nw16x2 = l16x2.waves_per_part;
            d.L1 = l1.L; d.nw1 = l1.waves_per_part;
            if ((rc = dev_alloc(g, l16.order.size(), &d.lst16, l16.order.data()))) return rc;
            if ((rc = dev_alloc(g, l16x2.order.size(), &d.lst16x2, l16x2.order.data()))) return rc;
            if ((rc = dev_alloc(g, l1.order.size(), &d.lst1, l1.order.data()))) return rc;
        }
    }
    if ((rc = dev_alloc(g, (size_t)g->M + 1, &A.sptr, hc.sptr.data()))) return rc;
    if ((rc = dev_alloc(g, (size_t)g->N + 1, &At.sptr, hv.sptr.data()))) return rc;
    if ((rc = dev_alloc(g, (size_t)g->nnz * 2, &A.sent))) return rc;
    if ((rc = dev_alloc(g, (size_t)g->nnz * 2, &At.sent))) return rc;
    if ((rc = dev_alloc(g, (size_t)g->nnz * 2, &A.sax))) return rc;
    if ((rc = dev_alloc(g, (size_t)g->nnz * 2, &At.sax))) return rc;
    if ((rc = dev_alloc(g, (size_t)g->N, &g->inv_n_p))) return rc;
    if ((rc = dev_alloc(g, (size_t)g->N, &g->x1_p))) return rc;
    if ((rc = dev_alloc(g, (size_t)g->M, &g->x2_p))) return rc;
    if ((rc = dev_alloc(g, (size_t)g->N, &g->labels_p))) return rc;
    if (!g->tail_sync) {
        if ((rc = dev_alloc(g, (size_t)4, &g->tail_sync))) return rc;
        MLLP_HIP_TRY(hipMemset(g->tail_sync, 0, 32));
        MLLP_HIP_TRY(hipHostMalloc((void**)&g->tail_err_host, 64, hipHostMallocMapped));
        *g->tail_err_host = 0u;
        MLLP_HIP_TRY(hipHostGetDevicePointer((void**)&g->tail_err_dev, g->tail_err_host, 0));
    }
    if ((rc = fused_refill_values(g, 0))) return rc;
    if (g->N > 0) {
        hipLaunchKernelGGL(fused_permute_kernel, dim3(256), dim3(256), 0, 0, (int)g->N, g->perm_v, g->inv_n, g->inv_n_p);
        if ((rc = check_launch("fused_permute inv_n"))) return rc;
    }
    MLLP_HIP_TRY(hipDeviceSynchronize());
    g->fused_built = true;
    return MLLP_OK;
}

int fused_bind(mllp_graph* g, const float* x1, const float* x2, const float* labels, hipStream_t s) {
    int rc;
    hipStreamCaptureStatus cap = hipStreamCaptureStatusNone;
    (void)hipStreamIsCapturing(s, &cap);
    const bool capturing = cap != hipStreamCaptureStatusNone;
    if (capturing) g->bound_x1 = g->bound_x2 = g->bound_labels = nullptr;
    if (x1 != g->bound_x1 || x2 != g->bound_x2) {
        if (g->N > 0) hipLaunchKernelGGL(fused_permute_kernel, dim3(256), dim3(256), 0, s, (int)g->N, g->perm_v, x1, g->x1_p);
        if (g->M > 0) hipLaunchKernelGGL(fused_permute_kernel, dim3(256), dim3(256), 0, s, (int)g->M, g->perm_c, x2, g->x2_p);
        if (g->nnz > 0) {
            hipLaunchKernelGGL(fused_pregather_kernel, dim3(1024), dim3(256), 0, s, g->nnz,
                               reinterpret_cast<const int2*>(g->FA.sent), g->x1_p, reinterpret_cast<float2*>(g->FA.sax));
            hipLaunchKernelGGL(fused_pregather_kernel, dim3(1024), dim3(256), 0, s, g->nnz,
                               reinterpret_cast<const int2*>(g->FAt.sent), g->x2_p, reinterpret_cast<float2*>(g->FAt.sax));
        }
        if ((rc = check_launch("fused_bind inputs"))) return rc;
        if (!capturing) { g->bound_x1 = x1; g->bound_x2 = x2; }
    }
    if (labels && labels != g->bound_labels) {
        if (g->N > 0) hipLaunchKernelGGL(fused_permute_kernel, dim3(256), dim3(256), 0, s, (int)g->N, g->perm_v, labels, g->labels_p);
        if ((rc = check_launch("fused_bind labels"))) return rc;
        if (!capturing) g->bound_labels = labels;
    }
    return MLLP_OK;
}

int fused_grid(const mllp_graph* g) { return std::max(std::min(g->n_cu, STAT_BLOCKS_MAX) / NP, 1) * NP; }

static FwdJob16 fwd_job16(const FusedOrient& o, const float* cp, const ConvWs& w, const float* x_src, const float* x_dst,
                          float* h) {
    FwdJob16 J = {};
    J.s = items_dev(o, 0);
    J.x_src = x_src; J.x_dst = x_dst; J.D = w.derived; J.p = conv_params_at(cp, 16);
    J.h = h; J.Z = w.Z; J.aux = w.aux;
    J.head = 0;
#ifdef MLLP_TIMING_BUILD
    J.abl = g_fused_abl;
#endif
    return J;
}
static FwdJob1 fwd_job1(const FusedOrient& o, const float* cp, const ConvWs& w, const float* x_dst, float* h) {
    FwdJob1 J = {};
    J.s = items_dev(o, 1);
    J.x_dst = x_dst; J.D = w.derived; J.p = conv_params_at(cp, 1);
    J.h = h; J.Z = w.Z; J.aux = w.aux;
    return J;
}

int fused_forward(mllp_graph* g, const FusedModel& m, int head_mode, hipStream_t s, bool skip_prep) {
    const int G = fused_grid(g);
    int rc;
    if ((rc = fused_bind(g, m.x1, m.x2, head_mode == 2 ? m.labels : nullptr, s))) return rc;
    if (!skip_prep) {
        const float* cps[MODEL_CONVS] = {m.cp[0], m.cp[1], m.cp[2], m.cp[3], m.cp[4]};
        const int cins[MODEL_CONVS] = {1, 1, 16, 16, 16};
        float* ders[MODEL_CONVS] = {m.c[0].derived, m.c[1].derived, m.c[2].derived, m.c[3].derived, m.c[4].derived};
        if ((rc = launch_param_prep_batch(MODEL_CONVS, cps, cins, ders, s))) return rc;
    }
    {
        FwdLaunch1 L = {};
        L.n_jobs = 2;
        L.job[0] = fwd_job1(g->FAt, m.cp[0], m.c[0], g->x1_p, m.h1v);
        L.job[1] = fwd_job1(g->FA, m.cp[1], m.c[1], g->x2_p, m.h1c);
        hipLaunchKernelGGL(fused_fwd1_kernel, dim3(G), dim3(FT), 0, s, L);
        if ((rc = check_launch("fused_fwd1"))) return rc;
    }
    {
        FwdLaunch16 L = {};
        L.n_jobs = 2;
        L.job[0] = fwd_job16(g->FAt, m.cp[2], m.c[2], m.h1c, m.h1v, m.h2v);
        L.job[1] = fwd_job16(g->FA, m.cp[3], m.c[3], m.h1v, m.h1c, m.h2c);
        L.job[0].perm = g->perm_v; L.job[1].perm = g->perm_c;
        hipLaunchKernelGGL(fused_fwd16_kernel, dim3(G), dim3(FT), 0, s, L);
        if ((rc = check_launch("fused_fwd16 layer 2"))) return rc;
    }
    {
        FwdLaunch16 L = {};
        L.n_jobs = 1;
        L.job[0] = fwd_job16(g->FAt, m.cp[4], m.c[4], m.h2c, m.h2v, m.h3v);
        FwdJob16& J = L.job[0];
        J.head = head_mode;
        J.fcw = m.fcw; J.fcb = m.fcb; J.inv_n = g->inv_n_p; J.labels = g->labels_p; J.perm = g->perm_v;
        J.inv_batch = m.inv_batch;
        J.logits = m.logits; J.g_out = m.d3v; J.head_part = m.head_part;
        hipLaunchKernelGGL(fused_fwd16_kernel, dim3(G), dim3(FT), 0, s, L);
        if ((rc = check_launch("fused_fwd16 layer 3"))) return rc;
    }
    return MLLP_OK;
}

int fused_head_backward(const mllp_graph* g, const FusedModel& m, const float* dlogits, hipStream_t s) {
    const int G = fused_grid(g);
    hipLaunchKernelGGL(fused_head_bwd_kernel, dim3(G), dim3(RT), 0, s, (int)g->N, m.h3v, m.fcw, dlogits, g->perm_v, m.d3v,
                       m.head_part);
    return check_launch("fused_head_bwd");
}

static BwdJob16 bwd_job16(const FusedOrient& o, const float* cp, const ConvWs& w, const float* x_src, const float* x_dst,
                          const float* h, const float* dh_a, const float* dh_b, float* dx_dst, bool need_rec, bool mask_dx) {
    BwdJob16 J = {};
    J.s = items_dev(o, 0);
    J.x_src = x_src; J.x_dst = x_dst; J.D = w.derived; J.p = conv_params_at(cp, 16);
    J.h = h; J.dh_a = dh_a; J.dh_b = dh_b; J.Z = w.Z; J.aux = w.aux;
    J.rec = need_rec ? w.rec : nullptr;
    J.dx_dst = dx_dst;
    J.mask_dx = mask_dx ? 1 : 0;
    J.stats = w.stats;
#ifdef MLLP_TIMING_BUILD
    J.abl = g_fused_abl;
#endif
    return J;
}
static SrcJob16 src_job16(const FusedOrient& o_src_major, const ConvWs& w, const float* x_rows, float* dx, const float* add) {
    SrcJob16 J = {};
    J.s = items_dev(o_src_major, 2);
    J.x = x_rows; J.rec = w.rec; J.dx = dx;
    J.addp = add ? add : x_rows; J.addw = add ? 1.0f : 0.0f; J.mask = 1;
    return J;
}
static BwdJob1 bwd_job1(const FusedOrient& o, const float* cp, const ConvWs& w, const float* x_dst, const float* g_masked) {
    BwdJob1 J = {};
    J.s = items_dev(o, 1);
    J.x_dst = x_dst; J.D = w.derived; J.p = conv_params_at(cp, 1);
    J.g = g_masked; J.Z = w.Z; J.aux = w.aux; J.stats = w.stats;
    return J;
}

int fused_backward(const mllp_graph* g, const FusedModel& m, bool premasked, float* grads, float* loss, hipStream_t s,
                   const FusedAdam* adam) {
    const int G = fused_grid(g);
    int rc;
    const FusedOrient& A = g->FA;
    const FusedOrient& At = g->FAt;
    {
        BwdLaunch16 L = {};
        L.n_jobs = 1;
        L.job[0] = bwd_job16(At, m.cp[4], m.c[4], m.h2c, m.h2v, premasked ? nullptr : m.h3v, m.d3v, nullptr, m.d2v, true, true);
        hipLaunchKernelGGL(fused_bwd16_kernel, dim3(G), dim3(FT), 0, s, L);
        if ((rc = check_launch("fused_bwd16 C3"))) return rc;
    }
    {
        SrcLaunch16 S = {};
        S.n_jobs = 1;
        S.job[0] = src_job16(A, m.c[4], m.h2c, m.d2c, nullptr);
        hipLaunchKernelGGL(fused_src16_kernel, dim3(2 * G), dim3(FT), 0, s, S);
        if ((rc = check_launch("fused_src16 C3"))) return rc;
        BwdLaunch16 L = {};
        L.n_jobs = 1;
        L.job[0] = bwd_job16(At, m.cp[2], m.c[2], m.h1c, m.h1v, nullptr, m.d2v, nullptr, m.d1v, true, true);
        hipLaunchKernelGGL(fused_bwd16_kernel, dim3(G), dim3(FT), 0, s, L);
        if ((rc = check_launch("fused_bwd16 C2V"))) return rc;
    }
    {
        BwdLaunch16 L = {};
        L.n_jobs = 1;
        L.job[0] = bwd_job16(A, m.cp[3], m.c[3], m.h1v, m.h1c, nullptr, m.d2c, nullptr, m.d1c, true, true);
        hipLaunchKernelGGL(fused_bwd16_kernel, dim3(G), dim3(FT), 0, s, L);
        if ((rc = check_launch("fused_bwd16 C2C"))) return rc;
        SrcLaunch16 S = {};
        S.n_jobs = 2;
        S.job[0] = src_job16(A, m.c[2], m.h1c, m.d1c_b, m.d1c);
        S.job[1] = src_job16(At, m.c[3], m.h1v, m.d1v_b, m.d1v);
        hipLaunchKernelGGL(fused_src16_kernel, dim3(2 * G), dim3(FT), 0, s, S);
        if ((rc = check_launch("fused_src16 C2V + C2C"))) return rc;
    }
    {
        BwdLaunch1 L = {};
        L.n_jobs = 2;
        L.job[0] = bwd_job1(A, m.cp[1], m.c[1], g->x2_p, m.d1c_b);
        L.job[1] = bwd_job1(At, m.cp[0], m.c[0], g->x1_p, m.d1v_b);
        hipLaunchKernelGGL(fused_bwd1_kernel, dim3(G), dim3(FT), 0, s, L);
        if ((rc = check_launch("fused_bwd1"))) return rc;
    }
    ReduceArgs R = {};
    for (int i = 0; i < MODEL_CONVS; ++i) { R.stats[i] = m.c[i].stats; R.out[i] = m.c[i].red; }
    R.nblk = G;
    R.head_part = m.have_head_part ? m.head_part : nullptr;
    R.head_out = grads + 4704;
    R.loss_out = loss;
    const int cins[MODEL_CONVS] = {1, 1, 16, 16, 16};
    float* grs[MODEL_CONVS] = {grads + 0, grads + 144, grads + 288, grads + 1392, grads + 2496};
    if (adam) {
        TailArgs T = {};
        T.R = R;
        for (int i = 0; i < MODEL_CONVS; ++i) {
            T.p[i] = conv_params_at(m.cp[i], cins[i]);
            T.cin[i] = cins[i];
            T.grads[i] = grs[i];
            T.D[i] = m.c[i].derived;
        }
        T.zero = grads + 3600;
        T.n_zero = 1104;
        T.params = adam->params; T.grads_all = grads; T.m = adam->m; T.v = adam->v; T.state = adam->state;
        T.eps = adam->eps;
        T.n_params = adam->n;
        T.sync = g->tail_sync;
        T.err = g->tail_err_dev;
        if (g->tail_err_host && *(volatile unsigned*)g->tail_err_host != 0u)
            return fail(MLLP_EHIP, "the grid barrier of fused_tail_kernel timed out in an earlier step (the device was shared with "
                                   "other work): parameters and optimizer state since then are invalid; recreate the graph");
        hipLaunchKernelGGL(fused_tail_kernel, dim3(MODEL_CONVS * STAT_TILES + 1), dim3(RT), 0, s, T, MODEL_CONVS);
        return check_launch("fused_tail");
    }
    {
        hipLaunchKernelGGL(fused_reduce_kernel, dim3(MODEL_CONVS * STAT_TILES + 1), dim3(RT), 0, s, R, MODEL_CONVS);
        if ((rc = check_launch("fused_reduce"))) return rc;
    }
    {
        const float* cps[MODEL_CONVS] = {m.cp[0], m.cp[1], m.cp[2], m.cp[3], m.cp[4]};
        const float* sts[MODEL_CONVS] = {m.c[0].red, m.c[1].red, m.c[2].red, m.c[3].red, m.c[4].red};
        const int nbs[MODEL_CONVS] = {1, 1, 1, 1, 1};
        if ((rc = launch_finalize_batch(MODEL_CONVS, cps, cins, sts, nbs, grs, grads + 3600, 1104, s))) return rc;
    }
    return MLLP_OK;
}

}
```

mllp_amd/csrc/host_graph.cpp:

```cpp
#include "host_graph.h"

#include <array>

#include <algorithm>
#include <atomic>
#include <thread>

#include "../../include/mllp_hip.h"

namespace mllp {

int host_build_batch(int64_t n_inst, const int64_t* inst_m, const int64_t* inst_n, const int64_t* indptr,
                     const int32_t* indices, const double* values, HostBatch* out, std::string* err,
                     unsigned max_threads) {
    auto bad_arg = [&](int code, const char* msg) {
        if (err) *err = msg;
        return code;
    };
    if (!out) return bad_arg(MLLP_EINVAL, "host_build_batch: out is null");
    if (n_inst < 0 || (n_inst > 0 && (!inst_m || !inst_n || !indptr)))
        return bad_arg(MLLP_EINVAL, "mllp_graph_create_host: null instance arrays");
    std::vector<int64_t> pm(n_inst + 1, 0), pn(n_inst + 1, 0), pe(n_inst + 1, 0), pp(n_inst + 1, 0);
    for (int64_t k = 0; k < n_inst; ++k) {
        if (inst_m[k] < 0 || inst_n[k] < 0) return bad_arg(MLLP_EINVAL, "negative instance size");
        pm[k + 1] = pm[k] + inst_m[k];
        pn[k + 1] = pn[k] + inst_n[k];
        pp[k + 1] = pp[k] + inst_m[k] + 1;
        const int64_t* ip = indptr + pp[k];
        if (ip[0] != 0) return bad_arg(MLLP_EINVAL, "indptr block does not start at 0");
        if (ip[inst_m[k]] < 0) return bad_arg(MLLP_EINVAL, "indptr not monotone");
        pe[k + 1] = pe[k] + ip[inst_m[k]];
    }
    const int64_t M = pm[n_inst], N = pn[n_inst], nnz = pe[n_inst];
    if (nnz >= INT32_MAX - 1 || M >= INT32_MAX - 1 || N >= INT32_MAX - 1)
        return bad_arg(MLLP_ERANGE, "batch exceeds int32 indexing");
    if (nnz > 0 && (!indices || !values)) return bad_arg(MLLP_EINVAL, "null indices/values");

    HostBatch& b = *out;
    b.M = M; b.N = N; b.nnz = nnz; b.n_inst = n_inst;
    b.csr_ptr.assign(M + 1, 0); b.csr_idx.assign(nnz, 0); b.csr_val.assign(nnz, 0.0f);
    b.csc_ptr.assign(N + 1, 0); b.csc_idx.assign(nnz, 0); b.csc_val.assign(nnz, 0.0f);
    std::atomic<int> bad{0};
    std::atomic<int64_t> next{0};
    auto worker = [&]() {
        std::vector<int> cnt;
        for (;;) {
            const int64_t k = next.fetch_add(1);
            if (k >= n_inst || bad.load()) break;
            const int64_t m = inst_m[k], n = inst_n[k], e0 = pe[k], e1 = pe[k + 1];
            const int64_t* ip = indptr + pp[k];
            const int32_t* ix = indices + e0;
            const double* va = values + e0;
            cnt.assign(n + 1, 0);
            bool ok = true;
            for (int64_t r = 0; r < m && ok; ++r) {
                if (ip[r + 1] < ip[r] || ip[r + 1] > e1 - e0) { bad = 1; ok = false; break; }
                b.csr_ptr[pm[k] + r + 1] = (int)(e0 + ip[r + 1]);
                int prev = -1;
                for (int64_t e = ip[r]; e < ip[r + 1]; ++e) {
                    const int c = ix[e];
                    if (c < 0 || c >= n || c <= prev) { bad = 2; ok = false; break; }
                    prev = c;
                    b.csr_idx[e0 + e] = (int)(pn[k] + c);
                    b.csr_val[e0 + e] = (float)va[e];
                    cnt[c + 1]++;
                }
            }
            if (!ok) break;
            for (int64_t c = 0; c < n; ++c) cnt[c + 1] += cnt[c];
            for (int64_t c = 0; c < n; ++c) b.csc_ptr[pn[k] + c + 1] = (int)(e0 + cnt[c + 1]);
            for (int64_t r = 0; r < m; ++r)
                for (int64_t e = ip[r]; e < ip[r + 1]; ++e) {
                    const int c = ix[e];
                    const int64_t pos = e0 + cnt[c]++;
                    b.csc_idx[pos] = (int)(pm[k] + r);
                    b.csc_val[pos] = (float)va[e];
                }
        }
    };
    unsigned nt = max_threads ? max_threads : std::max(1u, std::min(16u, std::thread::hardware_concurrency()));
    nt = (unsigned)std::min<int64_t>(nt, std::max<int64_t>(n_inst, 1));
    std::vector<std::thread> th;
    for (unsigned i = 1; i < nt; ++i) th.emplace_back(worker);
    worker();
    for (auto& t : th) t.join();
    if (bad == 1) return bad_arg(MLLP_EINVAL, "indptr not monotone");
    if (bad == 2) return bad_arg(MLLP_EINVAL, "column ids must be in range, sorted and unique within a row");
    b.pm = std::move(pm);
    b.pn = std::move(pn);
    return MLLP_OK;
}

TierConfig host_choose_tiers(int64_t nnz, int tier_wave, int tier_block) {
    const bool throughput = nnz >= (int64_t)32 << 20;
    TierConfig c;
    c.tier_wave = tier_wave > 0 ? tier_wave : (throughput ? 1024 : 64);
    c.tier_block = tier_block > 0 ? tier_block : (throughput ? 16384 : 256);
    if (c.tier_block < c.tier_wave) c.tier_block = c.tier_wave;
    c.chunk_nnz = 4 * c.tier_block;
    return c;
}

void host_build_tiers(const int* ptr, int n_dst, const TierConfig& cfg, HostTiers* out) {
    HostTiers& t = *out;
    t = HostTiers();
    int slots = 0;
    for (int r = 0; r < n_dst; ++r) {
        const int beg = ptr[r], end = ptr[r + 1], deg = end - beg;
        if (deg > cfg.tier_block) {
            const int nck = (deg + cfg.chunk_nnz - 1) / cfg.chunk_nnz;
            if (nck == 1) {
                t.chunks.insert(t.chunks.end(), {r, beg, end, -1});
            } else {
                t.split.insert(t.split.end(), {r, slots, nck, 0});
                const int per = ((deg + nck - 1) / nck + 255) & ~255;
                for (int c = 0; c < nck; ++c) {
                    const int cb = std::min(beg + c * per, end), ce = std::min(cb + per, end);
                    t.chunks.insert(t.chunks.end(), {r, cb, ce, slots++});
                }
            }
        } else if (deg > cfg.tier_wave) {
            t.rows_wave.push_back(r);
        } else {
            t.n_group++;
        }
    }
    t.n_slots = slots;
    t.short_rows = n_dst > 0 && (double)ptr[n_dst] / n_dst <= 16.0;
}

std::vector<int64_t> host_instance_cost(const int* ptr, const std::vector<int64_t>& inst_off) {
    constexpr int64_t ITEM = FUSED_COST_ITEM, STEP = FUSED_COST_STEP;
    const size_t n = inst_off.empty() ? 0 : inst_off.size() - 1;
    std::vector<int64_t> cost(n, 0);
    for (size_t k = 0; k < n; ++k) {
        int64_t c = 0;
        for (int64_t r = inst_off[k]; r < inst_off[k + 1]; ++r) {
            const int64_t deg = ptr[r + 1] - ptr[r];
            if (deg > FUSED_T16[2]) c += 12 * FUSED_COST_BLOCK_ROW;
            else if (deg > FUSED_T16[1]) c += ITEM + STEP * ((deg + 63) / 64);
            else if (deg > FUSED_T16[0]) c += (ITEM + STEP * ((deg + 15) / 16)) / 4;
            else c += (ITEM + STEP * ((deg + 3) / 4)) / 16;
        }
        cost[k] = c;
    }
    return cost;
}

std::vector<InstLoad> host_instance_loads(const int* ptr, const std::vector<int64_t>& inst_off) {
    const size_t n = inst_off.empty() ? 0 : inst_off.size() - 1;
    std::vector<InstLoad> out(n);
    for (size_t k = 0; k < n; ++k) {
        InstLoad& l = out[k];
        for (int64_t r = inst_off[k]; r < inst_off[k + 1]; ++r) {
            const int64_t deg = ptr[r + 1] - ptr[r];
            if (deg > FUSED_T16[2]) { l.d[0] += 16 * FUSED_BLOCK_ROW_ITEMS; l.d[1] += 16 * 2 * ((deg + 767) / 768); l.d[4] += 1; }
            else if (deg > FUSED_T16[1]) { l.d[0] += 16; l.d[1] += 16 * ((deg + 63) / 64); }
            else if (deg > FUSED_T16[0]) { l.d[0] += 4; l.d[1] += 4 * ((deg + 15) / 16); }
            else { l.d[0] += 1; l.d[1] += std::max<int64_t>((deg + 3) / 4, 1); }
            if (deg > FUSED_T1[2]) { l.d[2] += 64 * FUSED_BLOCK_ROW_ITEMS; l.d[3] += 64 * 2 * ((deg + 6143) / 6144); }
            else if (deg > FUSED_T1[1]) { l.d[2] += 64; l.d[3] += 64 * ((deg + 511) / 512); }
            else if (deg > FUSED_T1[0]) { l.d[2] += 4; l.d[3] += 4 * ((deg + 31) / 32); }
            else { l.d[2] += 1; l.d[3] += std::max<int64_t>((deg + 7) / 8, 1); }
            if (deg > FUSED_T16[2]) l.d[5] += 12 * FUSED_COST_BLOCK_ROW;
            else if (deg > FUSED_T16[1]) l.d[5] += FUSED_COST_ITEM + FUSED_COST_STEP * ((deg + 63) / 64);
            else if (deg > FUSED_T16[0]) l.d[5] += (FUSED_COST_ITEM + FUSED_COST_STEP * ((deg + 15) / 16)) / 4;
            else l.d[5] += (FUSED_COST_ITEM + FUSED_COST_STEP * ((deg + 3) / 4)) / 16;
        }
    }
    return out;
}

namespace {
struct VecBalance {
    static constexpr int D = 2 * FUSED_LOAD_DIMS;
    int n_parts;
    std::vector<std::array<double, D>> x;
    std::vector<std::array<double, D>> load;
    double max_of(int q) const {
        double m = 0.0;
        for (int d = 0; d < D; ++d) m = std::max(m, load[(size_t)q][d]);
        return m;
    }
    double worst() const {
        double m = 0.0;
        for (int q = 0; q < n_parts; ++q) m = std::max(m, max_of(q));
        return m;
    }
};
}

double host_partition_imbalance(const std::vector<InstLoad>& a, const std::vector<InstLoad>& b, const std::vector<int>& part,
                                int n_parts) {
    double worst = 0.0;
    for (int side = 0; side < 2; ++side)
        for (int d = 0; d < FUSED_LOAD_DIMS; ++d) {
            if (d == 4) continue;
            std::vector<double> l((size_t)n_parts, 0.0);
            double tot = 0.0;
            for (size_t i = 0; i < a.size(); ++i) {
                const double v = (double)(side ? b[i].d[d] : a[i].d[d]);
                l[(size_t)part[i]] += v;
                tot += v;
            }
            if (tot <= 0.0) continue;
            for (int q = 0; q < n_parts; ++q) worst = std::max(worst, l[(size_t)q] * n_parts / tot);
        }
    return worst;
}

std::vector<int> host_partition_instances_v(const std::vector<InstLoad>& a, const std::vector<InstLoad>& b, int n_parts) {
    const int n = (int)a.size();
    constexpr int D = VecBalance::D;
    VecBalance vb;
    vb.n_parts = n_parts;
    vb.x.assign((size_t)n, std::array<double, D>{});
    vb.load.assign((size_t)n_parts, std::array<double, D>{});
    double tot[D] = {};
    for (int i = 0; i < n; ++i)
        for (int d = 0; d < FUSED_LOAD_DIMS; ++d) { tot[d] += (double)a[i].d[d]; tot[FUSED_LOAD_DIMS + d] += (double)b[i].d[d]; }
    std::vector<double> size((size_t)n, 0.0);
    for (int i = 0; i < n; ++i)
        for (int d = 0; d < D; ++d) {
            const double v = (double)(d < FUSED_LOAD_DIMS ? a[i].d[d] : b[i].d[d - FUSED_LOAD_DIMS]);
            vb.x[(size_t)i][d] = tot[d] > 0.0 && d % FUSED_LOAD_DIMS != 4 ? v * n_parts / tot[d] : 0.0;
            size[(size_t)i] = std::max(size[(size_t)i], vb.x[(size_t)i][d]);
        }
    std::vector<int> order((size_t)n), part((size_t)n, 0);
    for (int i = 0; i < n; ++i) order[(size_t)i] = i;
    std::stable_sort(order.begin(), order.end(), [&](int p, int q) { return size[(size_t)p] > size[(size_t)q]; });
    std::vector<int> count((size_t)n_parts, 0);
    for (int i : order) {
        int best = 0;
        double best_v = 0.0;
        for (int q = 0; q < n_parts; ++q) {
            double v = 0.0;
            for (int d = 0; d < D; ++d) v = std::max(v, vb.load[(size_t)q][d] + vb.x[(size_t)i][d]);
            if (q == 0 || v < best_v - 1e-12 || (v < best_v + 1e-12 && count[(size_t)q] < count[(size_t)best])) { best = q; best_v = v; }
        }
        part[(size_t)i] = best;
        count[(size_t)best]++;
        for (int d = 0; d < D; ++d) vb.load[(size_t)best][d] += vb.x[(size_t)i][d];
    }
    if (n <= 4096) {
        for (int round = 0; round < 200; ++round) {
            int wq = 0;
            for (int q = 1; q < n_parts; ++q)
                if (vb.max_of(q) > vb.max_of(wq)) wq = q;
            const double cur = vb.max_of(wq);
            double best_gain = 1e-9;
            int bi = -1, bj = -1, bq = -1;
            auto pair_max = [&](int q1, int q2, int i, int j) {
                double m = 0.0;
                for (int d = 0; d < D; ++d) {
                    const double xi = vb.x[(size_t)i][d], xj = j >= 0 ? vb.x[(size_t)j][d] : 0.0;
                    m = std::max(m, std::max(vb.load[(size_t)q1][d] - xi + xj, vb.load[(size_t)q2][d] + xi - xj));
                }
                return m;
            };
            for (int i = 0; i < n; ++i) {
                if (part[(size_t)i] != wq) continue;
                for (int q = 0; q < n_parts; ++q) {
                    if (q == wq) continue;
                    const double m0 = pair_max(wq, q, i, -1);
                    if (cur - m0 > best_gain) { best_gain = cur - m0; bi = i; bj = -1; bq = q; }
                    for (int j = 0; j < n; ++j) {
                        if (part[(size_t)j] != q) continue;
                        const double m1 = pair_max(wq, q, i, j);
                        if (cur - m1 > best_gain) { best_gain = cur - m1; bi = i; bj = j; bq = q; }
                    }
                }
            }
            if (bi < 0) break;
            for (int d = 0; d < D; ++d) {
                const double xi = vb.x[(size_t)bi][d], xj = bj >= 0 ? vb.x[(size_t)bj][d] : 0.0;
                vb.load[(size_t)wq][d] += xj - xi;
                vb.load[(size_t)bq][d] += xi - xj;
            }
            part[(size_t)bi] = bq;
            if (bj >= 0) part[(size_t)bj] = wq;
        }
    }
    std::vector<int64_t> ca((size_t)n), cb((size_t)n);
    for (int i = 0; i < n; ++i) { ca[(size_t)i] = a[(size_t)i].d[5]; cb[(size_t)i] = b[(size_t)i].d[5]; }
    const std::vector<int> alt = host_partition_instances(ca, cb, n_parts);
    return host_partition_imbalance(a, b, alt, n_parts) < host_partition_imbalance(a, b, part, n_parts) - 1e-12 ? alt : part;
}

std::vector<int> host_partition_instances(const std::vector<int64_t>& cost_a, const std::vector<int64_t>& cost_b, int n_parts) {
    const int n = (int)cost_a.size();
    std::vector<int64_t> ca((size_t)n), cb((size_t)n);
    int64_t sa = 1, sb = 1;
    for (int i = 0; i < n; ++i) {
        ca[i] = cost_a[i] + 1;
        cb[i] = cost_b[i] + 1;
        sa += ca[i]; sb += cb[i];
    }
    std::vector<int> order((size_t)n), part((size_t)n, 0);
    for (int i = 0; i < n; ++i) order[i] = i;
    std::stable_sort(order.begin(), order.end(), [&](int a, int b) { return ca[a] + cb[a] > ca[b] + cb[b]; });
    std::vector<int64_t> la((size_t)n_parts, 0), lb((size_t)n_parts, 0);
    for (int i : order) {
        int best = 0;
        double best_v = 0.0;
        for (int q = 0; q < n_parts; ++q) {
            const double v = std::max((double)(la[q] + ca[i]) / (double)sa, (double)(lb[q] + cb[i]) / (double)sb);
            if (q == 0 || v < best_v) { best = q; best_v = v; }
        }
        part[i] = best;
        la[best] += ca[i];
        lb[best] += cb[i];
    }
    return part;
}

void host_build_fused_orient(const int* ptr, int n, const std::vector<int64_t>& inst_off, const std::vector<int>& inst_part,
                             HostFusedOrient* out) {
    HostFusedOrient& o = *out;
    o = HostFusedOrient();
    n = std::max(n, 0);
    o.perm.resize((size_t)n);
    o.inv.resize((size_t)n);
    o.sptr.assign((size_t)n + 1, 0);
    std::vector<int> node_part((size_t)n, 0);
    for (size_t k = 0; k + 1 < inst_off.size(); ++k)
        for (int64_t r = inst_off[k]; r < inst_off[k + 1] && r < n; ++r) node_part[(size_t)r] = inst_part[k];
    for (int r = 0; r < n; ++r) o.perm[r] = r;
    std::stable_sort(o.perm.begin(), o.perm.end(), [&](int a, int b) {
        if (node_part[a] != node_part[b]) return node_part[a] < node_part[b];
        return ptr[a + 1] - ptr[a] > ptr[b + 1] - ptr[b];
    });
    for (int q = 0; q <= FUSED_PARTS; ++q) o.row0[q] = 0;
    for (int k = 0; k < n; ++k) {
        const int r = o.perm[k], deg = ptr[r + 1] - ptr[r], q = node_part[r];
        o.inv[r] = k;
        o.sptr[k + 1] = o.sptr[k] + deg;
        o.row0[q + 1]++;
        for (int which = 0; which < 2; ++which) {
            const int(&T)[3] = which ? FUSED_T1 : FUSED_T16;
            FusedTiers& t = which ? o.t1[q] : o.t16[q];
            if (deg > T[2]) t.n_block++;
            else if (deg > T[1]) t.n_wave++;
            else if (deg > T[0]) t.n_group++;
            else t.n_base++;
        }
    }
    for (int q = 0; q < FUSED_PARTS; ++q) o.row0[q + 1] += o.row0[q];
}

void host_build_wave_lists(const HostFusedOrient& o, bool scalar, int waves_per_part, int waves_per_wg, int nnz_per_step,
                           HostWaveLists* out) {
    HostWaveLists& wl = *out;
    wl = HostWaveLists();
    const int nw = std::max(waves_per_part, 1), wpg = std::max(std::min(waves_per_wg, nw), 1), gp = std::max(nw / wpg, 1);
    wl.waves_per_part = nw;
    const int U = scalar ? 64 : 16, RG = U / 4;
    const int e_base = std::max(nnz_per_step, 1), e_group = 4 * e_base, e_wave = (scalar ? 64 : 16) * e_base;
    std::vector<std::vector<int>> lists((size_t)FUSED_PARTS * nw);
    for (int q = 0; q < FUSED_PARTS; ++q) {
        const FusedTiers& t = scalar ? o.t1[q] : o.t16[q];
        const int n_gitems = (t.n_group + RG - 1) / RG, n_bitems = (t.n_base + U - 1) / U;
        const int n_items = t.n_wave + n_gitems + n_bitems;
        auto deg_of = [&](int rl) { const int k = o.row0[q] + rl; return (int64_t)o.sptr[(size_t)k + 1] - o.sptr[(size_t)k]; };
        std::vector<std::pair<int64_t, int>> items((size_t)n_items);
        for (int it = 0; it < n_items; ++it) {
            int64_t steps;
            if (it < t.n_wave) steps = (deg_of(t.n_block + it) + e_wave - 1) / e_wave;
            else if (it < t.n_wave + n_gitems) steps = (deg_of(t.n_block + t.n_wave + (it - t.n_wave) * RG) + e_group - 1) / e_group;
            else steps = (deg_of(t.n_block + t.n_wave + t.n_group + (it - t.n_wave - n_gitems) * U) + e_base - 1) / e_base;
            items[(size_t)it] = {FUSED_COST_ITEM + FUSED_COST_STEP * std::max<int64_t>(steps, 1), it};
        }
        std::stable_sort(items.begin(), items.end(), [](const auto& a, const auto& b) { return a.first > b.first; });
        std::vector<int64_t> load((size_t)nw, 0), slow((size_t)nw, 0);
        for (int w = 0; w < nw; ++w) {
            const int bi = w / wpg;
            const int n_rows = bi < gp && t.n_block > bi ? (t.n_block - bi + gp - 1) / gp : 0;
            slow[(size_t)w] = 1000 + 95 * ((w % wpg) / 4);
            load[(size_t)w] = FUSED_COST_BLOCK_ROW * n_rows * slow[(size_t)w] / 1000;
        }
        for (const auto& itc : items) {
            int best = 0;
            int64_t best_t = 0;
            for (int w = 0; w < nw; ++w) {
                const int64_t tw = load[(size_t)w] + itc.first * slow[(size_t)w] / 1000;
                if (w == 0 || tw < best_t) { best = w; best_t = tw; }
            }
            lists[(size_t)q * nw + best].push_back(itc.second);
            load[(size_t)best] = best_t;
        }
        for (int w = 0; w < nw; ++w) {
            wl.max_load = std::max(wl.max_load, load[(size_t)w]);
            wl.sum_load += load[(size_t)w];
            wl.L = std::max(wl.L, (int)lists[(size_t)q * nw + w].size());
        }
    }
    wl.L = std::max(wl.L, 1);
    wl.order.assign((size_t)FUSED_PARTS * nw * wl.L, -1);
    for (size_t k = 0; k < lists.size(); ++k) std::copy(lists[k].begin(), lists[k].end(), wl.order.begin() + k * wl.L);
}

}
```

mllp_amd/csrc/host_graph.h:

```cpp
#pragma once
#include <stdint.h>

#include <string>
#include <vector>

namespace mllp {

struct HostBatch {
    int64_t M = 0, N = 0, nnz = 0, n_inst = 0;
    std::vector<int64_t> pm, pn;
    std::vector<int> csr_ptr, csr_idx;
    std::vector<float> csr_val;
    std::vector<int> csc_ptr, csc_idx;
    std::vector<float> csc_val;
};

int host_build_batch(int64_t n_inst, const int64_t* inst_m, const int64_t* inst_n, const int64_t* indptr,
                     const int32_t* indices, const double* values, HostBatch* out, std::string* err,
                     unsigned max_threads = 0);

struct TierConfig {
    int tier_wave = 0, tier_block = 0, chunk_nnz = 0;
};
TierConfig host_choose_tiers(int64_t nnz, int tier_wave, int tier_block);

struct HostTiers {
    std::vector<int> rows_wave;
    std::vector<int> chunks;
    std::vector<int> split;
    int n_group = 0, n_slots = 0;
    bool short_rows = false;
};
void host_build_tiers(const int* ptr, int n_dst, const TierConfig& cfg, HostTiers* out);

constexpr int FUSED_PARTS = 8;
struct FusedTiers {
    int n_block = 0, n_wave = 0, n_group = 0, n_base = 0;
};
struct HostFusedOrient {
    std::vector<int> perm;
    std::vector<int> inv;
    std::vector<int> sptr;
    int row0[FUSED_PARTS + 1];
    FusedTiers t16[FUSED_PARTS], t1[FUSED_PARTS];
};
constexpr int FUSED_T16[3] = {16, 64, 1024};
constexpr int FUSED_T1[3] = {16, 64, 4096};
constexpr int64_t FUSED_COST_ITEM = 5300, FUSED_COST_STEP = 2000, FUSED_COST_BLOCK_ROW = 25000;
std::vector<int64_t> host_instance_cost(const int* ptr, const std::vector<int64_t>& inst_off);
std::vector<int> host_partition_instances(const std::vector<int64_t>& cost_a, const std::vector<int64_t>& cost_b, int n_parts);
constexpr int FUSED_BLOCK_ROW_ITEMS = 10;
constexpr int FUSED_LOAD_DIMS = 6;
struct InstLoad {
    int64_t d[FUSED_LOAD_DIMS] = {0, 0, 0, 0, 0, 0};
};
std::vector<InstLoad> host_instance_loads(const int* ptr, const std::vector<int64_t>& inst_off);
std::vector<int> host_partition_instances_v(const std::vector<InstLoad>& a, const std::vector<InstLoad>& b, int n_parts);
double host_partition_imbalance(const std::vector<InstLoad>& a, const std::vector<InstLoad>& b, const std::vector<int>& part,
                                int n_parts);
void host_build_fused_orient(const int* ptr, int n, const std::vector<int64_t>& inst_off, const std::vector<int>& inst_part,
                             HostFusedOrient* out);
struct HostWaveLists {
    std::vector<int> order;
    int L = 0, waves_per_part = 0;
    int64_t max_load = 0, sum_load = 0;
};
void host_build_wave_lists(const HostFusedOrient& o, bool scalar, int waves_per_part, int waves_per_wg, int nnz_per_step,
                           HostWaveLists* out);

}
```

mllp_amd/csrc/internal.h:

```cpp
#pragma once
#include <hip/hip_runtime.h>
#include <stdint.h>

#include <algorithm>
#include <string>
#include <vector>

#include "../../include/mllp_hip.h"

namespace mllp {

constexpr int FEAT = 16;
constexpr int BLOCK = 256;
constexpr int REC_W = 40;
constexpr int STAT_TILES = 7;
constexpr int STAT_FLOATS = STAT_TILES * 256;
constexpr int STAT_BLOCKS_MAX = 256;

void set_error(const std::string& msg);
int fail(int code, const std::string& msg);
int hip_fail(hipError_t e, const char* what);

#define MLLP_HIP_TRY(expr)                                              \
    do {                                                                \
        hipError_t _e = (expr);                                         \
        if (_e != hipSuccess) return ::mllp::hip_fail(_e, #expr);       \
    } while (0)

template <class T>
struct DevBuf {
    T* p = nullptr;
    ~DevBuf() { if (p) (void)hipFree(p); }
    int alloc(size_t n) { return hipMalloc((void**)&p, std::max<size_t>(n, 1) * sizeof(T)) == hipSuccess ? 0 : 1; }
};

struct Tiled {
    int n_tiles = 0, n_tb = 0, max_nbt = 0, max_run = 0;
    bool owned = false;
    const int* tile_blk = nullptr;
    const int* blk_id = nullptr;
    const int* ptr2 = nullptr;
    const int* perm = nullptr;
    const int* ent = nullptr;
    int* vmap = nullptr;
};
constexpr int TILED_SPMM = 0;
constexpr int TILED_ATTN = 1;
constexpr int TILED_BSRC = 2;
constexpr int TILED_SCALAR = 3;
constexpr int TILED_BDST = 4;
constexpr int TILED_VARIANTS = 5;

struct StreamCopy {
    int n_tiles = 0, n_tb = 0;
    int64_t n_groups = 0;
    int64_t step_slots = 0;
    int* tile_row = nullptr;
    int* tile_blk = nullptr;
    int* blk_id = nullptr;
    int* rows = nullptr;
    int* hdr = nullptr;
    int* ent = nullptr;
    int* vmap = nullptr;
    double build_seconds = 0.0;
};

struct LaneCopy {
    int n_tiles = 0, n_tb = 0;
    int64_t n_groups = 0;
    int64_t nnz = 0;
    int* tile_row = nullptr;
    int* tile_blk = nullptr;
    int* tile_col = nullptr;
    int* rows = nullptr;
    int* whdr = nullptr;
    unsigned* offs = nullptr;
    float* vals = nullptr;
    int* vmap = nullptr;
    double build_seconds = 0.0;
};

struct CopyArray {
    void** p;
    int64_t bytes;
};
enum { SC_TILE_BLK, SC_BLK_ID, SC_ROWS, SC_ENT, SC_TILE_ROW, SC_HDR };
enum { LC_TILE_BLK, LC_TILE_COL, LC_ROWS, LC_OFFS, LC_TILE_ROW, LC_WHDR, LC_VALS };
enum { TL_TILE_BLK, TL_BLK_ID, TL_PTR2, TL_PERM, TL_ENT };
std::vector<CopyArray> stream_copy_arrays(StreamCopy& sc, int geom);
std::vector<CopyArray> lane_copy_arrays(LaneCopy& lc);
std::vector<CopyArray> tiled_arrays(Tiled& tl, int variant, int64_t nnz);
int copy_alloc(const CopyArray& a);
void copy_free(const std::vector<CopyArray>& arrays);

struct Orient {
    LaneCopy lane1;
    StreamCopy stream[4];
    Tiled tiled[TILED_VARIANTS];
    int n_dst = 0, n_src = 0;
    int* ptr = nullptr;
    int* idx = nullptr;
    float* val = nullptr;
    int* rows_group = nullptr;
    int* rows_wave = nullptr;
    int* chunks = nullptr;
    int* split = nullptr;
    int n_group = 0, n_wave = 0, n_chunk = 0, n_split = 0, n_slots = 0;
    float* scratch = nullptr;
    int tier_wave = 0;
    bool short_rows = false;
};
struct FusedTiersDev {
    int n_block = 0, n_wave = 0, n_group = 0, n_base = 0;
};
constexpr int FUSED_NP = 8;
struct FusedOrient {
    int n_dst = 0, n_src = 0, nnz = 0;
    int* sptr = nullptr;
    int* sent = nullptr;
    float* sax = nullptr;
    int row0[FUSED_NP + 1] = {};
    FusedTiersDev t16[FUSED_NP], t1[FUSED_NP];
    int* lst16 = nullptr; int* lst16x2 = nullptr; int* lst1 = nullptr;
    int L16 = 0, L16x2 = 0, L1 = 0, nw16 = 0, nw16x2 = 0, nw1 = 0;
};
constexpr int SCRATCH_NS = 20;

}

struct mllp_graph {
    int64_t M = 0, N = 0, nnz = 0, n_inst = 0;
    mllp::Orient A;
    mllp::Orient At;
    float* inv_n = nullptr;
    int* inst_ptr_n = nullptr;
    int* inst_ptr_m = nullptr;
    std::vector<int64_t> h_inst_ptr_n, h_inst_ptr_m;
    std::vector<int> h_csr_ptr, h_csc_ptr;
    int tier_wave = 0, tier_block = 0, chunk_nnz = 0;
    int max_inst_n = 0;
    int n_cu = 256;
    int path = 0;
    bool fused_built = false;
    mllp::FusedOrient FA, FAt;
    int* perm_v = nullptr;
    int* perm_c = nullptr;
    int* inv_v = nullptr;
    int* inv_c = nullptr;
    float* inv_n_p = nullptr;
    unsigned long long* tail_sync = nullptr;
    unsigned* tail_err_host = nullptr;
    unsigned* tail_err_dev = nullptr;
    float* x1_p = nullptr;
    float* x2_p = nullptr;
    float* labels_p = nullptr;
    const void* bound_x1 = nullptr;
    const void* bound_x2 = nullptr;
    const void* bound_labels = nullptr;
    int ws_path = -1;
    const void* ws_ptr = nullptr;
    const void* folded_ws = nullptr;
    const void* folded_params = nullptr;
    int* at_pos = nullptr;
    float* scale_buf = nullptr;
    hipStream_t aux = nullptr;
    hipEvent_t ev[16] = {};
    std::vector<void*> allocs;
};

namespace mllp {

struct ConvParams {
    const float *Wk, *bk, *Wq, *bq, *Wv, *bv, *we, *Ws, *bs;
};
inline int conv_param_count(int cin) { return 4 * FEAT * cin + 5 * FEAT; }
inline ConvParams conv_params_at(const float* base, int cin) {
    ConvParams p;
    const float* q = base;
    p.Wk = q; q += FEAT * cin;
    p.bk = q; q += FEAT;
    p.Wq = q; q += FEAT * cin;
    p.bq = q; q += FEAT;
    p.Wv = q; q += FEAT * cin;
    p.bv = q; q += FEAT;
    p.we = q; q += FEAT;
    p.Ws = q; q += FEAT * cin;
    p.bs = q;
    return p;
}

constexpr int OFF_PQ = 0, OFF_PQT = 256, OFF_WST = 512, OFF_WVT = 768;
constexpr int OFF_PQ0 = 1024, OFF_PT = 1040, OFF_PB = 1056, OFF_PT0 = 1072;
constexpr int DERIVED_W = 1088;

struct ConvWs {
    float* derived;
    float* qp;
    float* t;
    float* Z;
    float* aux;
    float* rec;
    float* dqp;
    float* dsdt;
    float* stats;
    float* red;
};
int64_t conv_ws_floats(int64_t n_dst, int cin);
ConvWs conv_ws_carve(float* base, int64_t n_dst, int cin);

int launch_spmm(const Orient& o, const float* H, float* Y, float* scratch, hipStream_t s);
int build_stream_device(const Orient& o, int64_t nnz, const std::vector<int>& tile_row, StreamCopy& sc, hipStream_t s,
                        int geom = 0);
void stream_copy_free(StreamCopy& sc);
int build_tiled_device(const Orient& o, int64_t nnz, int variant, Tiled& out, hipStream_t s);
void tiled_free(Tiled& tl);
int launch_spmm_stream(const StreamCopy& sc, int n_dst, int n_src, const float* H, float* Y, hipStream_t s);
struct ConvWs;
int launch_fwd16_stream(const StreamCopy& sc, int n_dst, int n_src, const float* conv_params, const ConvWs& w,
                        const float* x_src, const float* x_dst, float* h_out, hipStream_t s);
int launch_bwddst16_stream(const StreamCopy& sc, int n_dst, int n_src, const ConvWs& w, const float* x_src, const float* g,
                           float* dx_dst, int accumulate, hipStream_t s);
struct ConvWs;
int launch_fwd1_lane(const LaneCopy& lc, int n_dst, int n_src, const float* conv_params, const ConvWs& w, const float* x_src,
                     const float* x_dst, float* h_out, hipStream_t s);
int launch_bwddst1_lane(const LaneCopy& lc, int n_dst, int n_src, const ConvWs& w, const float* x_src, hipStream_t s);
int build_lane_copy(const Orient& o, int64_t nnz, const std::vector<int64_t>& seg, LaneCopy& lc, hipStream_t s);
void lane_copy_free(LaneCopy& lc);
int launch_bwdsrc16_stream(const StreamCopy& sc, int n_rows, int n_cols, const float* rec, const float* x_rows, float* dx,
                           int accumulate, hipStream_t s);
int launch_spmm_tiled(const Tiled& tl, int n_dst, int n_src, const float* H, float* Y, hipStream_t s);
int launch_spmm_tiled_bf16(const Tiled& tl, int n_dst, int n_src, const void* H_bf16, float* Y, hipStream_t s);
struct ConvWs;
int launch_fwd16_tiled(const Tiled& tl, int n_dst, int n_src, const float* conv_params, const ConvWs& w,
                       const float* x_src, const float* x_dst, float* h_out, hipStream_t s);
int launch_fwd1_tiled(const Tiled& tl, int n_dst, int n_src, const float* conv_params, const ConvWs& w,
                      const float* x_src, const float* x_dst, float* h_out, hipStream_t s);
int launch_bwddst1_tiled(const Tiled& tl, int n_dst, int n_src, const ConvWs& w, const float* x_src, hipStream_t s);
int launch_bwddst16_tiled(const Tiled& tl, int n_dst, int n_src, const ConvWs& w, const float* x_src, const float* g,
                          float* dx_dst, int accumulate, hipStream_t s);
int launch_bwdsrc16_tiled(const Tiled& tl, int n_rows, int n_cols, const float* rec, const float* x_rows, float* dx,
                          int accumulate, hipStream_t s);
int tiled_geometry(int variant, int* rows_per_tile, int* cols_per_block, int* bundle_capacity);
int tiled_max_blocks_per_tile();
constexpr int MODEL_CONVS = 5;
int launch_param_prep_batch(int n, const float* const* conv_params, const int* cin, float* const* derived, hipStream_t s);
int launch_finalize_batch(int n, const float* const* conv_params, const int* cin, const float* const* stats,
                          const int* n_stat_blocks, float* const* grads, float* zero, int n_zero, hipStream_t s);
int launch_param_prep(const float* conv_params, int cin, float* derived, hipStream_t s);
int launch_node_qp(const float* x_dst, int64_t n_dst, const float* derived, float* qp, float* t, hipStream_t s);
int launch_attn_fwd(const Orient& o, int cin, const float* conv_params, const ConvWs& w, const float* x_src,
                    const float* x_dst, float* h_out, float* scratch, hipStream_t s);
int launch_bwd_pre(int64_t n_dst, int cin, const float* conv_params, const ConvWs& w, const float* x_dst,
                   const float* h_out, float* dh, hipStream_t s);
int launch_attn_bwd_dst(const Orient& o, int cin, const float* conv_params, const ConvWs& w, const float* x_src,
                        const float* g, float* dx_dst, int accumulate, float* scratch, hipStream_t s);
int launch_attn_bwd_src(const Orient& o_src_major, const ConvWs& w, const float* x_src, float* dx_src,
                        int accumulate, float* scratch, hipStream_t s);
int launch_attn_bwd_src1(const Orient& o_src_major, const ConvWs& w, const float* x_src, float* dx_src,
                         int accumulate, float* scratch, hipStream_t s);
int launch_edge_grad(const Orient& o, int64_t nnz, int cin, const ConvWs& w, const float* x_src, const int* pos, float* dval,
                     int accumulate, hipStream_t s);
int build_csc_to_csr(const mllp_graph* g, int* pos, hipStream_t s);
int ensure_at_pos(mllp_graph* g, hipStream_t s);
int launch_layer1_dst_grads(const ConvWs& wv, const float* gv, float* dx1, int64_t n, const ConvWs& wc, const float* gc,
                            float* dx2, int64_t m, hipStream_t s);
int launch_param_stats(int cin, int64_t n_dst, const ConvWs& w, const float* x_dst, const float* g, hipStream_t s);
int launch_finalize_conv(int cin, const float* conv_params, const float* stats, int n_stat_blocks, float* grads,
                         hipStream_t s);
int stat_blocks_for(int64_t n_dst);

int launch_head(int mode, int64_t n, const float* h3v, const float* fc_w, const float* fc_b, const float* inv_n,
                const float* labels, float inv_batch, const float* dlogits_in, float* logits, float* dh3v,
                float* partials, hipStream_t s);
int launch_head_finalize(const float* partials, int n_blocks, float* grad_fc , float* loss ,
                         hipStream_t s);
int head_blocks_for(int64_t n);
int launch_adam(float* p, const float* g, float* m, float* v, float* state, float eps, float gscale, int64_t n,
                hipStream_t s);
int launch_fill_zero(float* p, int64_t n, hipStream_t s);
int launch_topm_metrics(const mllp_graph* g, const float* logits, const float* labels, void* scratch, float* out,
                        hipStream_t s);
int launch_topm_select(const int* ptr_n, const int* ptr_m, int64_t n_seg, int n_dense, int m_dense, const float* logits,
                       unsigned char* mask, int* index, float* stats, hipStream_t s);

struct FusedModel {
    const float* cp[MODEL_CONVS];
    ConvWs c[MODEL_CONVS];
    const float *x1, *x2, *fcw, *fcb, *labels;
    float inv_batch;
    float *h1v, *h1c, *h2v, *h2c, *h3v;
    float *d3v, *d2v, *d2c, *d1v, *d1c, *d1v_b, *d1c_b;
    float *logits, *head_part;
    bool have_head_part;
};
int fused_graph_build(mllp_graph* g, const int* h_csr_ptr, const int* h_csc_ptr);
int fused_grid(const mllp_graph* g);
int fused_refill_values(mllp_graph* g, hipStream_t s);
int fused_bind(mllp_graph* g, const float* x1, const float* x2, const float* labels, hipStream_t s);
int fused_forward(mllp_graph* g, const FusedModel& m, int head_mode, hipStream_t s, bool skip_prep = false);
int fused_head_backward(const mllp_graph* g, const FusedModel& m, const float* dlogits, hipStream_t s);
struct FusedAdam {
    float *params, *m, *v, *state;
    float eps;
    int n;
};
int fused_backward(const mllp_graph* g, const FusedModel& m, bool premasked, float* grads, float* loss, hipStream_t s,
                   const FusedAdam* adam = nullptr);

}
```

Before: 289,200 instances/s.

## Schedule block rows and wave items jointly per launch with a cost model

Block-tier rows were previously strided round-robin across workgroups. They are now assigned on the host by a greedy cost model, stored per workgroup, and read from device lists. Wave item lists are built per launch family and cover all jobs in that launch together. The model accounts for block-row cost, workgroup barriers, per-wave slowdown and per-family cost parameters. The aim is to reduce load imbalance and tail time across the fused SpMM kernels, in exchange for more host preprocessing and an extra indirection load per block row. Timing probes are also added, but only in the timing build.

```diff
diff --git a/mllp_amd/csrc/fused_kernels.hip b/mllp_amd/csrc/fused_kernels.hip
--- a/mllp_amd/csrc/fused_kernels.hip
+++ b/mllp_amd/csrc/fused_kernels.hip
@@ -13,6 +13,10 @@
 #ifdef MLLP_TIMING_BUILD
 static int g_fused_abl = [] {
     const char* e = getenv("MLLP_FUSED_ABL");
+    return e ? atoi(e) : 0;
+}();
+static int g_fused_legacy_lists = [] {
+    const char* e = getenv("MLLP_FUSED_LEGACY_LISTS");
     return e ? atoi(e) : 0;
 }();
 #define FUSED_ABL(bit) ((J.abl & (bit)) != 0)
@@ -26,9 +30,39 @@
         stamp_sum[k] += now_ - stamp_last;                                                  \
         stamp_last = now_;                                                                  \
     }
+__device__ unsigned long long g_fused_wave[5][8192 * 8];
+struct WaveProbe {
+    unsigned long long t0, tb, tj, v[8];
+};
+#define PROBE_DECL WaveProbe pb = {}; pb.t0 = __builtin_amdgcn_s_memtime();
+#define PROBE_JOB_BEGIN pb.tj = __builtin_amdgcn_s_memtime();
+#define PROBE_BLOCK_BEGIN pb.tb = __builtin_amdgcn_s_memtime();
+#define PROBE_BLOCK_ROW(E, r) { pb.v[3] += 1; pb.v[4] += probe_steps<E>(r); }
+#define PROBE_BLOCK_END pb.v[5] += __builtin_amdgcn_s_memtime() - pb.tb;
+#define PROBE_ITEM(E, r) { pb.v[1] += 1; pb.v[2] += probe_steps<E>(r); }
+#define PROBE_JOB_END(j)                                                      \
+    {                                                                         \
+        const unsigned long long now_ = __builtin_amdgcn_s_memtime();         \
+        pb.v[7] += now_ - pb.tj;                                              \
+        if ((j) == 0) pb.v[6] = now_ - pb.t0;                                 \
+    }
+#define PROBE_STORE(fam)                                                                                   \
+    if ((threadIdx.x & 63) == 0 && blockIdx.x * FW + (threadIdx.x >> 6) < 8192) {                         \
+        pb.v[0] = __builtin_amdgcn_s_memtime() - pb.t0;                                                    \
+        unsigned long long* d_ = g_fused_wave[fam] + (size_t)(blockIdx.x * FW + (threadIdx.x >> 6)) * 8;   \
+        for (int k_ = 0; k_ < 8; ++k_) d_[k_] = pb.v[k_];                                                  \
+    }
 #else
 #define FUSED_ABL(bit) false
 #define FUSED_STAMP(k)
+#define PROBE_DECL
+#define PROBE_JOB_BEGIN
+#define PROBE_BLOCK_BEGIN
+#define PROBE_BLOCK_ROW(E, r)
+#define PROBE_BLOCK_END
+#define PROBE_ITEM(E, r)
+#define PROBE_JOB_END(j)
+#define PROBE_STORE(fam)
 #endif
 
 constexpr int FT = 768;
@@ -48,16 +82,18 @@
     const float2* __restrict__ sax;
     int n_dst, nnz;
     const int* __restrict__ order;
-    int nw, L;
+    const int* __restrict__ blk;
+    int nw, L, BL;
     PartTiers part[NP];
 };
 
-static ItemsDev items_dev(const FusedOrient& o, int which) {
-    const bool scalar = which == 1;
+static_assert(FUSED_FAMILIES == 5, "FusedOrient::lst");
+static ItemsDev items_dev(const FusedOrient& o, FusedFamily f) {
+    const bool scalar = FUSED_COSTS[f].scalar;
+    const FusedOrient::Lists& l = o.lst[f];
     ItemsDev d;
-    d.order = which == 0 ? o.lst16 : which == 1 ? o.lst1 : o.lst16x2;
-    d.nw = which == 0 ? o.nw16 : which == 1 ? o.nw1 : o.nw16x2;
-    d.L = which == 0 ? o.L16 : which == 1 ? o.L1 : o.L16x2;
+    d.order = l.order; d.blk = l.block_rows;
+    d.nw = l.nw; d.L = l.L; d.BL = l.BL;
     d.sptr = o.sptr;
     d.sent = reinterpret_cast<const int2*>(o.sent);
     d.sax = reinterpret_cast<const float2*>(o.sax);
@@ -215,10 +251,25 @@
 __device__ __forceinline__ int slot_count(const RowSlot& r) {
     return r.first < r.end ? (r.end - r.first + r.stride - 1) / r.stride : 0;
 }
+#ifdef MLLP_TIMING_BUILD
+template <int E>
+__device__ __forceinline__ unsigned probe_steps(const RowSlot& r) {
+    int n = slot_count(r);
+    for (int m = 32; m >= 1; m >>= 1) n = max(n, __shfl_xor(n, m, 64));
+    return (unsigned)max((n + E - 1) / E, 1);
+}
+#endif
 __device__ __forceinline__ RowSlot empty_slot() {
     RowSlot r;
     r.row = -1; r.first = 0; r.stride = 1; r.end = 0; r.mode = 0; r.writer = false;
     return r;
+}
+__device__ __forceinline__ int block_rows_of(const ItemsDev& S, const PartTiers& P, int bi) {
+    return P.n_block > 0 && (bi + 1) * FW <= S.nw ? S.BL : 0;
+}
+__device__ __forceinline__ int block_row(const ItemsDev& S, const PartTiers& P, int px, int bi, int k) {
+    const int r = S.blk[((size_t)px * (S.nw / FW) + bi) * S.BL + k];
+    return r >= 0 && r < P.n_block ? P.row0 + r : -1;
 }
 struct WaveList {
     const int* p;
@@ -546,9 +597,10 @@
 #else
 #define STAMP_ARGS
 #endif
-    const int px = blockIdx.x % NP, bi = blockIdx.x / NP, gp = gridDim.x / NP;
+    const int px = blockIdx.x % NP, bi = blockIdx.x / NP;
     const int gw = bi * FW + wave;
     float* head_part = nullptr;
+    PROBE_DECL
     for (int j = 0; j < A.n_jobs; ++j) {
         const FwdJob16& J = A.job[j];
         const PartTiers P = J.s.part[px];
@@ -556,14 +608,20 @@
         const RowSlot none = empty_slot();
         FwdPending pend;
         pend.row = -1;
-        for (int k = bi; k < P.n_block; k += gp) {
-            const RowSlot r = block_slot<4>(J.s, P.row0 + k, tid);
+        PROBE_JOB_BEGIN
+        PROBE_BLOCK_BEGIN
+        for (int kb = 0, nb = block_rows_of(J.s, P, bi); kb < nb; ++kb) {
+            const int krow = block_row(J.s, P, px, bi, kb);
+            if (krow < 0) break;
+            const RowSlot r = block_slot<4>(J.s, krow, tid);
+            PROBE_BLOCK_ROW(4, r)
             const float4 xd = ld4(J.x_dst + (size_t)r.row * 16 + 4 * part);
             int2 en = first_entries<4>(J.s, r, part);
             const int lrow = J.head ? J.perm[r.row] : 0;
             FwdNext nx;
             fwd16_row(J, Ws_[j], P, r, xd, en, lrow, empty_request(), -1, nx, pend, part, lane, merge_lds, tiles, ha STAMP_ARGS);
         }
+        PROBE_BLOCK_END
         WaveList wl = wave_list(J.s, px, gw);
         for (int c0 = 0; c0 < wl.L; c0 += 64) {
             wave_list_chunk(wl, c0, lane);
@@ -579,6 +637,7 @@
             for (int k = 0; it >= 0; ++k) {
                 const int it2 = wave_list_get(wl, k + 2);
                 FwdNext nx;
+                PROBE_ITEM(4, r)
                 fwd16_row(J, Ws_[j], P, r, xd, en, lrow, q1, it2, nx, pend, part, lane, merge_lds, tiles, ha STAMP_ARGS);
 #ifdef MLLP_TIMING_BUILD
                 stamp_sum[7] += 1;
@@ -588,7 +647,9 @@
             }
         }
         fwd16_flush(J, pend, part);
-    }
+        PROBE_JOB_END(j)
+    }
+    PROBE_STORE(FUSED_FWD16)
 #ifdef MLLP_TIMING_BUILD
     if (lane == 0 && A.job[0].abl >= 0) {
         stamp_sum[6] = __builtin_amdgcn_s_memtime() - stamp_begin;
@@ -754,13 +815,22 @@
         }
     }
     __syncthreads();
-    const int px = blockIdx.x % NP, bi = blockIdx.x / NP, gp = gridDim.x / NP;
+    const int px = blockIdx.x % NP, bi = blockIdx.x / NP;
     const int gw = bi * FW + wave;
+    PROBE_DECL
     for (int j = 0; j < A.n_jobs; ++j) {
         const FwdJob1& J = A.job[j];
         const PartTiers P = J.s.part[px];
-        for (int k = bi; k < P.n_block; k += gp)
-            fwd1_row(J, Ws_[j], block_slot<1>(J.s, P.row0 + k, tid), lane, merge_lds);
+        PROBE_JOB_BEGIN
+        PROBE_BLOCK_BEGIN
+        for (int kb = 0, nb = block_rows_of(J.s, P, bi); kb < nb; ++kb) {
+            const int krow = block_row(J.s, P, px, bi, kb);
+            if (krow < 0) break;
+            const RowSlot r = block_slot<1>(J.s, krow, tid);
+            PROBE_BLOCK_ROW(8, r)
+            fwd1_row(J, Ws_[j], r, lane, merge_lds);
+        }
+        PROBE_BLOCK_END
         WaveList wl = wave_list(J.s, px, gw);
         for (int c0 = 0; c0 < wl.L; c0 += 64) {
             wave_list_chunk(wl, c0, lane);
@@ -770,11 +840,14 @@
                 const int itn = wave_list_get(wl, k + 1);
                 const RowSlot r = slot_make(q);
                 q = item_request<1>(J.s, P, max(itn, 0), lane);
+                PROBE_ITEM(8, r)
                 fwd1_row(J, Ws_[j], r, lane, merge_lds);
                 it = itn;
             }
         }
-    }
+        PROBE_JOB_END(j)
+    }
+    PROBE_STORE(FUSED_FWD1)
 }
 
 struct BwdJob16 {
@@ -1003,8 +1076,9 @@
     }
     __syncthreads();
     float* tiles = tiles_ + wave * TB_N * TILE;
-    const int px = blockIdx.x % NP, bi = blockIdx.x / NP, gp = gridDim.x / NP;
+    const int px = blockIdx.x % NP, bi = blockIdx.x / NP;
     const int gw = bi * FW + wave;
+    PROBE_DECL
     for (int j = 0; j < A.n_jobs; ++j) {
         const BwdJob16& J = A.job[j];
         const PartTiers P = J.s.part[px];
@@ -1012,14 +1086,20 @@
 #pragma unroll
         for (int i = 0; i < STAT_TILES; ++i) acc[i] = splat4(0.0f);
         const RowSlot none = empty_slot();
-        for (int k = bi; k < P.n_block; k += gp) {
-            const RowSlot r = block_slot<4>(J.s, P.row0 + k, tid);
+        PROBE_JOB_BEGIN
+        PROBE_BLOCK_BEGIN
+        for (int kb = 0, nb = block_rows_of(J.s, P, bi); kb < nb; ++kb) {
+            const int krow = block_row(J.s, P, px, bi, kb);
+            if (krow < 0) break;
+            const RowSlot r = block_slot<4>(J.s, krow, tid);
+            PROBE_BLOCK_ROW(4, r)
             BwdRow rd;
             bwd16_fetch(J, r, part, rd);
             int2 en = first_entries<4>(J.s, r, part);
             RowSlot rn;
             bwd16_row(J, Ws_[j], P, r, rd, en, -1, rn, part, lane, merge_lds, tiles, acc);
         }
+        PROBE_BLOCK_END
         WaveList wl = wave_list(J.s, px, gw);
         for (int c0 = 0; c0 < wl.L; c0 += 64) {
             wave_list_chunk(wl, c0, lane);
@@ -1031,11 +1111,13 @@
             for (int k = 0; it >= 0; ++k) {
                 const int itn = wave_list_get(wl, k + 1);
                 RowSlot rn;
+                PROBE_ITEM(4, r)
                 bwd16_row(J, Ws_[j], P, r, rd, en, itn, rn, part, lane, merge_lds, tiles, acc);
                 r = rn;
                 it = itn;
             }
         }
+        PROBE_JOB_END(j)
         __syncthreads();
         float* red = tiles_;
 #pragma unroll
@@ -1051,6 +1133,7 @@
             __syncthreads();
         }
     }
+    PROBE_STORE(FUSED_BWD16)
 }
 
 struct SrcJob16 {
@@ -1131,19 +1214,26 @@
 __global__ __launch_bounds__(FT) void fused_src16_kernel(SrcLaunch16 A) {
     __shared__ float merge_lds[FW * 20];
     const int tid = threadIdx.x, lane = tid & 63, wave = tid >> 6, part = lane & 3;
-    const int px = blockIdx.x % NP, bi = blockIdx.x / NP, gp = gridDim.x / NP;
+    const int px = blockIdx.x % NP, bi = blockIdx.x / NP;
     const int gw = bi * FW + wave;
+    PROBE_DECL
     for (int j = 0; j < A.n_jobs; ++j) {
         const SrcJob16& J = A.job[j];
         const PartTiers P = J.s.part[px];
         const RowSlot none = empty_slot();
-        for (int k = bi; k < P.n_block; k += gp) {
-            const RowSlot r = block_slot<4>(J.s, P.row0 + k, tid);
+        PROBE_JOB_BEGIN
+        PROBE_BLOCK_BEGIN
+        for (int kb = 0, nb = block_rows_of(J.s, P, bi); kb < nb; ++kb) {
+            const int krow = block_row(J.s, P, px, bi, kb);
+            if (krow < 0) break;
+            const RowSlot r = block_slot<4>(J.s, krow, tid);
+            PROBE_BLOCK_ROW(2, r)
             float4 xj = ld4(J.x + (size_t)r.row * 16 + 4 * part);
             int2 en = first_entries<2>(J.s, r, part);
             RowSlot rn;
             src16_row(J, r, xj, en, empty_request(), rn, part, lane, merge_lds);
         }
+        PROBE_BLOCK_END
         WaveList wl = wave_list(J.s, px, gw);
         for (int c0 = 0; c0 < wl.L; c0 += 64) {
             wave_list_chunk(wl, c0, lane);
@@ -1155,12 +1245,15 @@
                 const int itn = wave_list_get(wl, k + 1);
                 const SlotReq qn = itn >= 0 ? item_request<4>(J.s, P, itn, lane) : empty_request();
                 RowSlot rn;
+                PROBE_ITEM(2, r)
                 src16_row(J, r, xj, en, qn, rn, part, lane, merge_lds);
                 r = rn;
                 it = itn;
             }
         }
-    }
+        PROBE_JOB_END(j)
+    }
+    PROBE_STORE(FUSED_SRC16)
 }
 
 struct BwdJob1 {
@@ -1325,8 +1418,9 @@
     }
     __syncthreads();
     float* tiles = tiles_ + wave * TILE1;
-    const int px = blockIdx.x % NP, bi = blockIdx.x / NP, gp = gridDim.x / NP;
+    const int px = blockIdx.x % NP, bi = blockIdx.x / NP;
     const int gw = bi * FW + wave;
+    PROBE_DECL
 #ifdef MLLP_TIMING_BUILD
     unsigned long long stamp_sum[8] = {0, 0, 0, 0, 0, 0, 0, 0};
     unsigned long long stamp_last = __builtin_amdgcn_s_memtime();
@@ -1340,8 +1434,16 @@
         const PartTiers P = J.s.part[px];
         f32x4m accT = splat4(0.0f);
         float accS[6] = {0.0f, 0.0f, 0.0f, 0.0f, 0.0f, 0.0f};
-        for (int k = bi; k < P.n_block; k += gp)
-            bwd1_row(J, Ws_[j], block_slot<1>(J.s, P.row0 + k, tid), lane, merge_lds, tiles, accT, accS STAMP_ARGS1);
+        PROBE_JOB_BEGIN
+        PROBE_BLOCK_BEGIN
+        for (int kb = 0, nb = block_rows_of(J.s, P, bi); kb < nb; ++kb) {
+            const int krow = block_row(J.s, P, px, bi, kb);
+            if (krow < 0) break;
+            const RowSlot r = block_slot<1>(J.s, krow, tid);
+            PROBE_BLOCK_ROW(8, r)
+            bwd1_row(J, Ws_[j], r, lane, merge_lds, tiles, accT, accS STAMP_ARGS1);
+        }
+        PROBE_BLOCK_END
         WaveList wl = wave_list(J.s, px, gw);
         for (int c0 = 0; c0 < wl.L; c0 += 64) {
             wave_list_chunk(wl, c0, lane);
@@ -1351,6 +1453,7 @@
                 const int itn = wave_list_get(wl, k + 1);
                 const RowSlot r = slot_make(q);
                 q = item_request<1>(J.s, P, max(itn, 0), lane);
+                PROBE_ITEM(8, r)
                 bwd1_row(J, Ws_[j], r, lane, merge_lds, tiles, accT, accS STAMP_ARGS1);
 #ifdef MLLP_TIMING_BUILD
                 stamp_sum[7] += 1;
@@ -1358,6 +1461,7 @@
                 it = itn;
             }
         }
+        PROBE_JOB_END(j)
         __syncthreads();
         float* red = tiles_;
 #pragma unroll
@@ -1396,6 +1500,7 @@
     }
 #endif
 #undef STAMP_ARGS1
+    PROBE_STORE(FUSED_BWD1)
 }
 
 __global__ __launch_bounds__(RT) void fused_head_bwd_kernel(int n, const float* __restrict__ h3, const float* __restrict__ fcw,
@@ -1553,6 +1658,11 @@
 extern "C" int mllp_timing_read_stamps(unsigned long long* host, int n) {
     return hipMemcpyFromSymbol(host, HIP_SYMBOL(g_fused_stamps), (size_t)n * sizeof(unsigned long long)) == hipSuccess ? 0 : -1;
 }
+extern "C" int mllp_timing_read_wave(int family, unsigned long long* host, int n) {
+    if (family < 0 || family >= 5 || n < 0 || n > 8192 * 8) return -1;
+    return hipMemcpyFromSymbol(host, HIP_SYMBOL(g_fused_wave), (size_t)n * sizeof(unsigned long long),
+                               (size_t)family * 8192 * 8 * sizeof(unsigned long long)) == hipSuccess ? 0 : -1;
+}
 extern "C" int mllp_timing_read_stamps1(unsigned long long* host, int n) {
     return hipMemcpyFromSymbol(host, HIP_SYMBOL(g_fused_stamps1), (size_t)n * sizeof(unsigned long long)) == hipSuccess ? 0 : -1;
 }
@@ -1623,20 +1733,34 @@
     for (int q = 0; q <= NP; ++q) { A.row0[q] = hc.row0[q]; At.row0[q] = hv.row0[q]; }
     {
         const int gp = fused_grid(g) / NP;
-        const HostFusedOrient* ho[2] = {&hc, &hv};
-        FusedOrient* dv[2] = {&A, &At};
-        for (int k = 0; k < 2; ++k) {
-            HostWaveLists l16, l16x2, l1;
-            host_build_wave_lists(*ho[k], false, gp * FW, FW, 4, &l16);
-            host_build_wave_lists(*ho[k], false, 2 * gp * FW, FW, 2, &l16x2);
-            host_build_wave_lists(*ho[k], true, gp * FW, FW, 8, &l1);
-            FusedOrient& d = *dv[k];
-            d.L16 = l16.L; d.nw16 = l16.waves_per_part;
-            d.L16x2 = l16x2.L; d.nw16x2 = l16x2.waves_per_part;
-            d.L1 = l1.L; d.nw1 = l1.waves_per_part;
-            if ((rc = dev_alloc(g, l16.order.size(), &d.lst16, l16.order.data()))) return rc;
-            if ((rc = dev_alloc(g, l16x2.order.size(), &d.lst16x2, l16x2.order.data()))) return rc;
-            if ((rc = dev_alloc(g, l1.order.size(), &d.lst1, l1.order.data()))) return rc;
+        struct Launch { FusedFamily f; const HostFusedOrient* ho[2]; FusedOrient* dv[2]; int n; };
+        const Launch launches[] = {
+            {FUSED_FWD1, {&hv, &hc}, {&At, &A}, 2},
+            {FUSED_FWD16, {&hv, &hc}, {&At, &A}, 2},
+            {FUSED_BWD16, {&hv, nullptr}, {&At, nullptr}, 1},
+            {FUSED_BWD16, {&hc, nullptr}, {&A, nullptr}, 1},
+            {FUSED_SRC16, {&hc, &hv}, {&A, &At}, 2},
+            {FUSED_BWD1, {&hc, &hv}, {&A, &At}, 2},
+        };
+        for (const Launch& l : launches) {
+            const FusedCost& c = FUSED_COSTS[l.f];
+            const int nw = c.wgs_per_cu * gp * FW;
+            std::vector<const HostFusedOrient*> jobs(l.ho, l.ho + l.n);
+            std::vector<HostWaveLists> wl;
+#ifdef MLLP_TIMING_BUILD
+            if (g_fused_legacy_lists) {
+                wl.resize((size_t)l.n);
+                for (int j = 0; j < l.n; ++j) host_build_wave_lists(*jobs[(size_t)j], c.scalar, nw, FW, c.nnz_per_step, &wl[(size_t)j]);
+            } else
+#endif
+            host_build_launch_lists(jobs, c, nw, FW, &wl);
+            for (int j = 0; j < l.n; ++j) {
+                FusedOrient::Lists& d = l.dv[j]->lst[l.f];
+                const HostWaveLists& h = wl[(size_t)j];
+                d.L = h.L; d.nw = h.waves_per_part; d.BL = h.BL;
+                if ((rc = dev_alloc(g, h.order.size(), &d.order, h.order.data()))) return rc;
+                if ((rc = dev_alloc(g, h.block_rows.size(), &d.block_rows, h.block_rows.data()))) return rc;
+            }
         }
     }
     if ((rc = dev_alloc(g, (size_t)g->M + 1, &A.sptr, hc.sptr.data()))) return rc;
@@ -1697,7 +1821,7 @@
 static FwdJob16 fwd_job16(const FusedOrient& o, const float* cp, const ConvWs& w, const float* x_src, const float* x_dst,
                           float* h) {
     FwdJob16 J = {};
-    J.s = items_dev(o, 0);
+    J.s = items_dev(o, FUSED_FWD16);
     J.x_src = x_src; J.x_dst = x_dst; J.D = w.derived; J.p = conv_params_at(cp, 16);
     J.h = h; J.Z = w.Z; J.aux = w.aux;
     J.head = 0;
@@ -1708,7 +1832,7 @@
 }
 static FwdJob1 fwd_job1(const FusedOrient& o, const float* cp, const ConvWs& w, const float* x_dst, float* h) {
     FwdJob1 J = {};
-    J.s = items_dev(o, 1);
+    J.s = items_dev(o, FUSED_FWD1);
     J.x_dst = x_dst; J.D = w.derived; J.p = conv_params_at(cp, 1);
     J.h = h; J.Z = w.Z; J.aux = w.aux;
     return J;
@@ -1766,7 +1890,7 @@
 static BwdJob16 bwd_job16(const FusedOrient& o, const float* cp, const ConvWs& w, const float* x_src, const float* x_dst,
                           const float* h, const float* dh_a, const float* dh_b, float* dx_dst, bool need_rec, bool mask_dx) {
     BwdJob16 J = {};
-    J.s = items_dev(o, 0);
+    J.s = items_dev(o, FUSED_BWD16);
     J.x_src = x_src; J.x_dst = x_dst; J.D = w.derived; J.p = conv_params_at(cp, 16);
     J.h = h; J.dh_a = dh_a; J.dh_b = dh_b; J.Z = w.Z; J.aux = w.aux;
     J.rec = need_rec ? w.rec : nullptr;
@@ -1780,14 +1904,14 @@
 }
 static SrcJob16 src_job16(const FusedOrient& o_src_major, const ConvWs& w, const float* x_rows, float* dx, const float* add) {
     SrcJob16 J = {};
-    J.s = items_dev(o_src_major, 2);
+    J.s = items_dev(o_src_major, FUSED_SRC16);
     J.x = x_rows; J.rec = w.rec; J.dx = dx;
     J.addp = add ? add : x_rows; J.addw = add ? 1.0f : 0.0f; J.mask = 1;
     return J;
 }
 static BwdJob1 bwd_job1(const FusedOrient& o, const float* cp, const ConvWs& w, const float* x_dst, const float* g_masked) {
     BwdJob1 J = {};
-    J.s = items_dev(o, 1);
+    J.s = items_dev(o, FUSED_BWD1);
     J.x_dst = x_dst; J.D = w.derived; J.p = conv_params_at(cp, 1);
     J.g = g_masked; J.Z = w.Z; J.aux = w.aux; J.stats = w.stats;
     return J;
diff --git a/mllp_amd/csrc/host_graph.cpp b/mllp_amd/csrc/host_graph.cpp
--- a/mllp_amd/csrc/host_graph.cpp
+++ b/mllp_amd/csrc/host_graph.cpp
@@ -397,6 +397,147 @@
     wl.L = std::max(wl.L, 1);
     wl.order.assign((size_t)FUSED_PARTS * nw * wl.L, -1);
     for (size_t k = 0; k < lists.size(); ++k) std::copy(lists[k].begin(), lists[k].end(), wl.order.begin() + k * wl.L);
-}
-
-}
+    wl.wgs_per_part = gp;
+    for (int q = 0; q < FUSED_PARTS; ++q) wl.BL = std::max(wl.BL, ((scalar ? o.t1[q] : o.t16[q]).n_block + gp - 1) / gp);
+    wl.block_rows.assign((size_t)FUSED_PARTS * gp * wl.BL, -1);
+    for (int q = 0; q < FUSED_PARTS; ++q)
+        for (int k = 0; k < (scalar ? o.t1[q] : o.t16[q]).n_block; ++k)
+            wl.block_rows[((size_t)q * gp + k % gp) * wl.BL + k / gp] = k;
+}
+
+namespace {
+struct PartItems {
+    std::vector<std::pair<int64_t, int>> items;
+    std::vector<int64_t> item_cost;
+    std::vector<int64_t> block_cost;
+};
+PartItems part_items(const HostFusedOrient& o, const FusedCost& c, int q, int wpg) {
+    PartItems p;
+    const FusedTiers& t = c.scalar ? o.t1[q] : o.t16[q];
+    const int U = c.scalar ? 64 : 16, RG = U / 4;
+    const int e_base = std::max(c.nnz_per_step, 1), e_group = 4 * e_base, e_wave = U * e_base, e_block = wpg * e_wave;
+    const int n_gitems = (t.n_group + RG - 1) / RG, n_bitems = (t.n_base + U - 1) / U, n_items = t.n_wave + n_gitems + n_bitems;
+    auto deg_of = [&](int rl) { const int k = o.row0[q] + rl; return (int64_t)o.sptr[(size_t)k + 1] - o.sptr[(size_t)k]; };
+    p.items.resize((size_t)n_items);
+    p.item_cost.resize((size_t)n_items);
+    for (int it = 0; it < n_items; ++it) {
+        int64_t steps;
+        if (it < t.n_wave) steps = (deg_of(t.n_block + it) + e_wave - 1) / e_wave;
+        else if (it < t.n_wave + n_gitems) steps = (deg_of(t.n_block + t.n_wave + (it - t.n_wave) * RG) + e_group - 1) / e_group;
+        else steps = (deg_of(t.n_block + t.n_wave + t.n_group + (it - t.n_wave - n_gitems) * U) + e_base - 1) / e_base;
+        p.item_cost[(size_t)it] = c.item + c.step * std::max<int64_t>(steps, 1);
+        p.items[(size_t)it] = {p.item_cost[(size_t)it], it};
+    }
+    std::stable_sort(p.items.begin(), p.items.end(), [](const auto& a, const auto& b) { return a.first > b.first; });
+    p.block_cost.resize((size_t)t.n_block);
+    for (int k = 0; k < t.n_block; ++k) p.block_cost[(size_t)k] = c.block_row + c.block_step * ((deg_of(k) + e_block - 1) / e_block);
+    return p;
+}
+void wg_barrier(std::vector<int64_t>& load, int bi, int wpg) {
+    int64_t m = 0;
+    for (int w = bi * wpg; w < (bi + 1) * wpg; ++w) m = std::max(m, load[(size_t)w]);
+    for (int w = bi * wpg; w < (bi + 1) * wpg; ++w) load[(size_t)w] = m;
+}
+}
+
+void host_build_launch_lists(const std::vector<const HostFusedOrient*>& jobs, const FusedCost& c, int waves_per_part,
+                             int waves_per_wg, std::vector<HostWaveLists>* out) {
+    const int nw = std::max(waves_per_part, 1), wpg = std::max(std::min(waves_per_wg, nw), 1), gp = std::max(nw / wpg, 1);
+    const int n_jobs = (int)jobs.size();
+    out->assign((size_t)n_jobs, HostWaveLists());
+    std::vector<std::vector<std::vector<int>>> lists((size_t)n_jobs), brows((size_t)n_jobs);
+    for (int j = 0; j < n_jobs; ++j) {
+        lists[(size_t)j].resize((size_t)FUSED_PARTS * nw);
+        brows[(size_t)j].resize((size_t)FUSED_PARTS * gp);
+    }
+    std::vector<int64_t> slow((size_t)nw);
+    for (int w = 0; w < nw; ++w) slow[(size_t)w] = 1000 + c.slow * ((w % wpg) / 4);
+    for (int q = 0; q < FUSED_PARTS; ++q) {
+        std::vector<int64_t> load((size_t)nw, 0);
+        for (int j = 0; j < n_jobs; ++j) {
+            const PartItems p = part_items(*jobs[(size_t)j], c, q, wpg);
+            std::vector<int64_t> wg_free((size_t)gp, 0);
+            std::vector<char> wg_has((size_t)gp, 0);
+            for (int bi = 0; bi < gp; ++bi)
+                for (int w = bi * wpg; w < (bi + 1) * wpg; ++w) wg_free[(size_t)bi] = std::max(wg_free[(size_t)bi], load[(size_t)w]);
+            for (size_t k = 0; k < p.block_cost.size(); ++k) {
+                int best = 0;
+                for (int bi = 1; bi < gp; ++bi)
+                    if (wg_free[(size_t)bi] < wg_free[(size_t)best]) best = bi;
+                brows[(size_t)j][(size_t)q * gp + best].push_back((int)k);
+                wg_free[(size_t)best] += p.block_cost[k];
+                wg_has[(size_t)best] = 1;
+            }
+            for (int bi = 0; bi < gp; ++bi)
+                if (wg_has[(size_t)bi])
+                    for (int w = bi * wpg; w < (bi + 1) * wpg; ++w) load[(size_t)w] = wg_free[(size_t)bi];
+            for (const auto& itc : p.items) {
+                int best = 0;
+                int64_t best_t = 0;
+                for (int w = 0; w < nw; ++w) {
+                    const int64_t tw = load[(size_t)w] + itc.first * slow[(size_t)w] / 1000;
+                    if (w == 0 || tw < best_t) { best = w; best_t = tw; }
+                }
+                lists[(size_t)j][(size_t)q * nw + best].push_back(itc.second);
+                load[(size_t)best] = best_t;
+            }
+            if (c.job_barrier)
+                for (int bi = 0; bi < gp; ++bi) wg_barrier(load, bi, wpg);
+        }
+    }
+    for (int j = 0; j < n_jobs; ++j) {
+        HostWaveLists& wl = (*out)[(size_t)j];
+        wl.waves_per_part = nw;
+        wl.wgs_per_part = gp;
+        for (const auto& l : lists[(size_t)j]) wl.L = std::max(wl.L, (int)l.size());
+        wl.L = std::max(wl.L, 1);
+        wl.order.assign((size_t)FUSED_PARTS * nw * wl.L, -1);
+        for (size_t k = 0; k < lists[(size_t)j].size(); ++k)
+            std::copy(lists[(size_t)j][k].begin(), lists[(size_t)j][k].end(), wl.order.begin() + k * wl.L);
+        for (const auto& l : brows[(size_t)j]) wl.BL = std::max(wl.BL, (int)l.size());
+        wl.block_rows.assign((size_t)FUSED_PARTS * gp * wl.BL, -1);
+        for (size_t k = 0; k < brows[(size_t)j].size(); ++k)
+            std::copy(brows[(size_t)j][k].begin(), brows[(size_t)j][k].end(), wl.block_rows.begin() + k * wl.BL);
+    }
+    const LaunchLoad ll = host_model_launch(jobs, c, *out, waves_per_wg);
+    for (HostWaveLists& wl : *out) { wl.max_load = ll.max_load; wl.sum_load = ll.sum_load; }
+}
+
+LaunchLoad host_model_launch(const std::vector<const HostFusedOrient*>& jobs, const FusedCost& c,
+                             const std::vector<HostWaveLists>& lists, int waves_per_wg) {
+    LaunchLoad ll;
+    if (jobs.empty() || lists.size() != jobs.size()) return ll;
+    const int nw = std::max(lists[0].waves_per_part, 1), wpg = std::max(std::min(waves_per_wg, nw), 1), gp = std::max(nw / wpg, 1);
+    for (int q = 0; q < FUSED_PARTS; ++q) {
+        std::vector<int64_t> load((size_t)nw, 0);
+        for (size_t j = 0; j < jobs.size(); ++j) {
+            const HostWaveLists& wl = lists[j];
+            const PartItems p = part_items(*jobs[j], c, q, wpg);
+            for (int bi = 0; bi < gp && bi < wl.wgs_per_part; ++bi) {
+                int64_t cost = 0;
+                bool any = false;
+                for (int k = 0; k < wl.BL; ++k) {
+                    const int r = wl.block_rows[((size_t)q * wl.wgs_per_part + bi) * wl.BL + k];
+                    if (r >= 0 && r < (int)p.block_cost.size()) { cost += p.block_cost[(size_t)r]; any = true; }
+                }
+                if (!any) continue;
+                wg_barrier(load, bi, wpg);
+                for (int w = bi * wpg; w < (bi + 1) * wpg; ++w) load[(size_t)w] += cost;
+                ll.sum_load += cost * wpg;
+            }
+            for (int w = 0; w < nw; ++w)
+                for (int k = 0; k < wl.L; ++k) {
+                    const int it = wl.order[((size_t)q * nw + w) * wl.L + k];
+                    if (it < 0 || it >= (int)p.item_cost.size()) continue;
+                    load[(size_t)w] += p.item_cost[(size_t)it] * (1000 + c.slow * ((w % wpg) / 4)) / 1000;
+                    ll.sum_load += p.item_cost[(size_t)it];
+                }
+            if (c.job_barrier)
+                for (int bi = 0; bi < gp; ++bi) wg_barrier(load, bi, wpg);
+        }
+        for (int w = 0; w < nw; ++w) ll.max_load = std::max(ll.max_load, load[(size_t)w]);
+    }
+    return ll;
+}
+
+}
diff --git a/mllp_amd/csrc/host_graph.h b/mllp_amd/csrc/host_graph.h
--- a/mllp_amd/csrc/host_graph.h
+++ b/mllp_amd/csrc/host_graph.h
@@ -64,8 +64,35 @@
     std::vector<int> order;
     int L = 0, waves_per_part = 0;
     int64_t max_load = 0, sum_load = 0;
+    std::vector<int> block_rows;
+    int BL = 0, wgs_per_part = 0;
 };
 void host_build_wave_lists(const HostFusedOrient& o, bool scalar, int waves_per_part, int waves_per_wg, int nnz_per_step,
                            HostWaveLists* out);
 
+enum FusedFamily { FUSED_FWD16 = 0, FUSED_BWD16, FUSED_SRC16, FUSED_FWD1, FUSED_BWD1, FUSED_FAMILIES };
+struct FusedCost {
+    int64_t item, step;
+    int64_t block_row, block_step;
+    int64_t slow;
+    bool scalar;
+    int nnz_per_step;
+    int wgs_per_cu;
+    bool job_barrier;
+};
+constexpr FusedCost FUSED_COSTS[FUSED_FAMILIES] = {
+    {5300, 2000, 2500, 400, 95, false, 4, 1, false},
+    {5300, 2000, 2500, 400, 95, false, 4, 1, true},
+    {5300, 2000, 2500, 400, 95, false, 2, 2, false},
+    {5300, 2000, 2500, 400, 95, true, 8, 1, false},
+    {5300, 2000, 2500, 400, 95, true, 8, 1, true},
+};
+void host_build_launch_lists(const std::vector<const HostFusedOrient*>& jobs, const FusedCost& c, int waves_per_part,
+                             int waves_per_wg, std::vector<HostWaveLists>* out);
+struct LaunchLoad {
+    int64_t max_load = 0, sum_load = 0;
+};
+LaunchLoad host_model_launch(const std::vector<const HostFusedOrient*>& jobs, const FusedCost& c,
+                             const std::vector<HostWaveLists>& lists, int waves_per_wg);
+
 }
diff --git a/mllp_amd/csrc/internal.h b/mllp_amd/csrc/internal.h
--- a/mllp_amd/csrc/internal.h
+++ b/mllp_amd/csrc/internal.h
@@ -121,8 +121,12 @@
     float* sax = nullptr;
     int row0[FUSED_NP + 1] = {};
     FusedTiersDev t16[FUSED_NP], t1[FUSED_NP];
-    int* lst16 = nullptr; int* lst16x2 = nullptr; int* lst1 = nullptr;
-    int L16 = 0, L16x2 = 0, L1 = 0, nw16 = 0, nw16x2 = 0, nw1 = 0;
+    struct Lists {
+        int* order = nullptr;
+        int* block_rows = nullptr;
+        int L = 0, nw = 0, BL = 0;
+    };
+    Lists lst[5];
 };
 constexpr int SCRATCH_NS = 20;
 
```

Result: slower. 281,800 instances/s (-2.6%).
